# zju3dv/clean-pvnet

Measured on NVIDIA B200. Metric: ransac_vote_throughput, higher is better.
Workload: dtype f32

## Files before the change

### clean_pvnet_b200/_lib.py

```python
import ctypes
import os

_HERE = os.path.dirname(os.path.abspath(__file__))
LIB_PATH = os.path.join(_HERE, "libpvnet_vote_b200.so")

PVB_OK, PVB_ERR_INVALID, PVB_ERR_CUDA, PVB_ERR_WORKSPACE, PVB_ERR_CAPACITY, PVB_ERR_TIMEOUT = range(6)
PVB_HOST_STAGE_VERTEX, PVB_HOST_INPLACE_MASK = 2, 4
PVB_IPC_HANDLE_BYTES = 64
(PVB_MASK_U8, PVB_MASK_I8, PVB_MASK_I16, PVB_MASK_I32, PVB_MASK_I64, PVB_MASK_F32, PVB_MASK_F64) = range(7)
PVB_SELECT_BYTE, PVB_SELECT_EQ1 = 0, 1


class PvbDesc(ctypes.Structure):
    _fields_ = [
        ("B", ctypes.c_int32), ("H", ctypes.c_int32), ("W", ctypes.c_int32), ("K", ctypes.c_int32),
        ("hn", ctypes.c_int32),
        ("inlier_thresh", ctypes.c_float),
        ("min_num", ctypes.c_int32), ("max_num", ctypes.c_int32),
        ("mask_dtype", ctypes.c_int32), ("select_mode", ctypes.c_int32),
        ("mask_stride", ctypes.c_int64 * 3),
        ("vertex_stride", ctypes.c_int64 * 5),
        ("capacity", ctypes.c_int32), ("img_base", ctypes.c_int32),
        ("seed", ctypes.c_uint64),
        ("rng_tag_idx", ctypes.c_int32), ("rng_tag_sel", ctypes.c_int32),
    ]


class PvbLayout(ctypes.Structure):
    _fields_ = [(n, ctypes.c_size_t) for n in
                ("total", "status", "fgsum", "nz", "tn", "state", "bits", "ticket", "blocktot", "xy", "dirs", "hyp",
                 "counts", "win", "refit_partial", "refit_ticket")] + [
                    ("nwords", ctypes.c_int32), ("nblocks", ctypes.c_int32), ("capacity", ctypes.c_int32),
                    ("refit_splits", ctypes.c_int32)]


class PvbPnpOptions(ctypes.Structure):
    _fields_ = [("max_num_iterations", ctypes.c_int32), ("reserved", ctypes.c_int32),
                ("function_tolerance", ctypes.c_double), ("gradient_tolerance", ctypes.c_double),
                ("parameter_tolerance", ctypes.c_double)]


_vp, _i32, _sz, _f = ctypes.c_void_p, ctypes.c_int32, ctypes.c_size_t, ctypes.c_float
_dp, _lp = ctypes.POINTER(PvbDesc), ctypes.POINTER(PvbLayout)
SIGNATURES = {
    "pvb_version": (ctypes.c_int, []),
    "pvb_last_error": (ctypes.c_char_p, []),
    "pvb_workspace_bytes": (_sz, [_dp]),
    "pvb_workspace_layout": (ctypes.c_int, [_dp, _lp]),
    "pvb_ransac_voting_v3": (ctypes.c_int, [_dp, _vp, _vp, _vp, _vp, _vp, _vp, _sz, _vp]),
    "pvb_decode_v3": (ctypes.c_int, [_dp, _vp, _i32, ctypes.c_int64, _vp, _vp, _vp, _vp, _vp, _vp, _sz, _vp]),
    "pvb_estimate_voting_distribution": (ctypes.c_int, [_dp, _vp, _vp, _vp, _vp, _vp, _vp, _vp, _sz, _vp]),
    "pvb_uncertainty_weights": (ctypes.c_int, [_vp, _vp, _i32, _vp]),
    "pvb_uncertainty_pnp": (ctypes.c_int, [_vp, _vp, _vp, _vp, _vp, _vp, _vp, _i32, _i32, ctypes.c_int64, ctypes.c_int64,
                                           ctypes.c_void_p, _vp]),
    "pvb_uncertainty_pnp_from_votes": (ctypes.c_int, [_vp, _vp, _vp, _vp, _vp, _vp, _vp, _vp, _vp, _vp, _i32, _i32,
                                                      ctypes.c_int64, ctypes.c_int64, ctypes.c_void_p, _vp]),
    "pvb_uncertainty_pnp_init": (ctypes.c_int, [_vp, _vp, _vp, _vp, _vp, _i32, _i32, ctypes.c_int64, ctypes.c_int64, _vp]),
    "pvb_read_status": (ctypes.c_int, [_dp, _vp, _vp]),
    "pvb_host_scratch_bytes": (_sz, [_dp, _i32]),
    "pvb_ransac_voting_v3_host": (ctypes.c_int, [_dp, _vp, _vp, _vp, _i32, ctypes.c_uint32, _vp, _sz, _vp]),
    "pvb_exchange_create": (ctypes.c_int, [_i32, _i32, _i32, _sz, ctypes.POINTER(ctypes.c_void_p)]),
    "pvb_exchange_bytes_per_rank": (_sz, [_vp]),
    "pvb_exchange_base": (ctypes.c_void_p, [_vp]),
    "pvb_exchange_get_handle": (ctypes.c_int, [_vp, _vp]),
    "pvb_exchange_connect": (ctypes.c_int, [_vp, _vp]),
    "pvb_exchange_connect_ptrs": (ctypes.c_int, [_vp, ctypes.POINTER(ctypes.c_void_p)]),
    "pvb_ransac_voting_v3_push": (ctypes.c_int, [_dp, _vp, _vp, _vp, _vp, _vp, _vp, _sz, _vp, ctypes.c_uint64, _vp]),
    "pvb_estimate_voting_distribution_push": (ctypes.c_int, [_dp, _vp, _vp, _vp, _vp, _vp, _vp, _vp, _sz, _vp, ctypes.c_uint64, _vp]),
    "pvb_exchange_wait": (ctypes.c_int, [_vp, ctypes.c_uint64, _vp, _vp, ctypes.c_double, _vp]),
    "pvb_exchange_status": (ctypes.c_int, [_vp, _vp]),
    "pvb_exchange_destroy": (ctypes.c_int, [_vp]),
    "pvb_profile_enable": (ctypes.c_int, [_i32]),
    "pvb_profile_reset": (ctypes.c_int, []),
    "pvb_set_tuning": (ctypes.c_int, [_i32, _i32]),
    "pvb_profile_read": (ctypes.c_int, [ctypes.POINTER(ctypes.c_double), _i32]),
    "pvb_generate_hypothesis": (ctypes.c_int, [_vp, _vp, _vp, _vp, _i32, _i32, _i32, _vp]),
    "pvb_voting_for_hypothesis": (ctypes.c_int, [_vp, _vp, _vp, _vp, _i32, _i32, _i32, _f, _vp]),
    "pvb_generate_hypothesis_vanishing_point": (ctypes.c_int, [_vp, _vp, _vp, _vp, _i32, _i32, _i32, _vp]),
    "pvb_voting_for_hypothesis_vanishing_point": (ctypes.c_int, [_vp, _vp, _vp, _vp, _i32, _i32, _i32, _f, _vp]),
    "pvb_vote_count": (ctypes.c_int, [_vp, _vp, _vp, _vp, _i32, _i32, _i32, _f, _vp, _sz, _vp]),
    "pvb_vote_count_workspace_bytes": (_sz, [_i32, _i32, _i32]),
}

_LIB = None


def load():
    global _LIB
    if _LIB is None:
        if not os.path.exists(LIB_PATH):
            raise RuntimeError(
                f"{LIB_PATH} is missing: build it with `python clean_pvnet_b200/build.py` "
                "(or __graft_entry__.build()). There is no CPU/PyTorch fallback for this op.")
        lib = ctypes.CDLL(LIB_PATH)
        for name, (res, args) in SIGNATURES.items():
            fn = getattr(lib, name)
            fn.restype = res
            fn.argtypes = args
        _LIB = lib
        if os.environ.get("PVB_VOTE_VARIANT"):
            check(lib.pvb_set_tuning(0, int(os.environ["PVB_VOTE_VARIANT"])))
    return _LIB


def check(rc):
    if rc != PVB_OK:
        msg = load().pvb_last_error().decode("utf-8", "replace")
        raise RuntimeError(f"pvnet_vote_b200 error {rc}: {msg}")
```

### clean_pvnet_b200/csrc/api.cu

```cuda
#include <cmath>
#include <cstdarg>
#include <cstdio>
#include <cstring>
#include <new>
#include <vector>
#include "kernels.h"

using namespace pvb;

namespace {

thread_local char g_err[512] = "";

int fail(int code, const char *fmt, ...)
{
    va_list ap;
    va_start(ap, fmt);
    vsnprintf(g_err, sizeof(g_err), fmt, ap);
    va_end(ap);
    return code;
}

int cuda_fail(cudaError_t e, const char *what)
{
    return fail(PVB_ERR_CUDA, "%s: %s", what, cudaGetErrorString(e));
}

inline size_t align_up(size_t v, size_t a = 256) { return (v + a - 1) / a * a; }

struct ProfCall {
    cudaEvent_t ev[PVB_STAGE_COUNT + 1];
    bool head;
};
thread_local int g_prof_every = 0;
thread_local unsigned g_prof_tick = 0;
thread_local std::vector<ProfCall> g_prof_calls;
thread_local std::vector<cudaEvent_t> g_prof_pool;

cudaEvent_t prof_event()
{
    if (!g_prof_pool.empty()) { cudaEvent_t e = g_prof_pool.back(); g_prof_pool.pop_back(); return e; }
    cudaEvent_t e = nullptr;
    cudaEventCreate(&e);
    return e;
}

ProfCall *prof_begin(bool head)
{
    if (g_prof_every <= 0 || (g_prof_tick++ % (unsigned)g_prof_every) != 0) return nullptr;
    ProfCall pc;
    for (auto &e : pc.ev) e = prof_event();
    pc.head = head;
    g_prof_calls.push_back(pc);
    return &g_prof_calls.back();
}

inline void prof_start(ProfCall *pc, int stage, cudaStream_t st) { if (pc && stage == 0) cudaEventRecord(pc->ev[0], st); }
inline void prof_end(ProfCall *pc, int stage, cudaStream_t st) { if (pc) cudaEventRecord(pc->ev[stage + 1], st); }

int default_capacity(const pvb_desc *d)
{
    const long long HW = (long long)d->H * d->W;
    long long cap = d->capacity;
    if (cap <= 0) {
        const long long mn = d->max_num < 0 ? 0 : d->max_num;
        cap = mn + (long long)ceil(8.0 * sqrt((double)mn)) + 64;
    }
    if (cap > HW) cap = HW;
    cap = (cap + 31) / 32 * 32;
    return (int)cap;
}

int check_desc(const pvb_desc *d)
{
    if (!d) return fail(PVB_ERR_INVALID, "descriptor is NULL");
    if (d->B < 0 || d->H <= 0 || d->W <= 0 || d->K <= 0 || d->hn <= 0)
        return fail(PVB_ERR_INVALID, "bad shape B=%d H=%d W=%d K=%d hn=%d", d->B, d->H, d->W, d->K, d->hn);
    if ((long long)d->H * d->W > (1ll << 30)) return fail(PVB_ERR_INVALID, "image too large (H*W > 2^30)");
    if (d->B > 65535 || d->K > 65535) return fail(PVB_ERR_INVALID, "B and K must be <= 65535");
    if ((long long)d->K * ((d->hn + 511) / 512) > 65535) return fail(PVB_ERR_INVALID, "K*ceil(hn/512) must be <= 65535");
    if (d->mask_dtype < PVB_MASK_U8 || d->mask_dtype > PVB_MASK_F64) return fail(PVB_ERR_INVALID, "bad mask_dtype %d", d->mask_dtype);
    if (d->select_mode != PVB_SELECT_BYTE && d->select_mode != PVB_SELECT_EQ1)
        return fail(PVB_ERR_INVALID, "bad select_mode %d", d->select_mode);
    return PVB_OK;
}

int make_layout(const pvb_desc *d, pvb_layout *L)
{
    const int rc = check_desc(d);
    if (rc) return rc;
    const size_t B = (size_t)d->B, K = (size_t)d->K, hn = (size_t)d->hn;
    const int nwords = (int)(((long long)d->H * d->W + 31) / 32);
    const int nblocks = (nwords + 127) / 128;
    const int cap = default_capacity(d);
    const int splits = refit_splits_for(cap);
    size_t off = 0;
    auto take = [&](size_t bytes) { const size_t o = off; off = align_up(off + bytes); return o; };
    L->status = take(4 * sizeof(int));
    L->fgsum = take(B * sizeof(unsigned long long));
    L->nz = take(B * sizeof(int));
    L->tn = take(B * sizeof(int));
    L->state = take(B * sizeof(int));
    L->refit_ticket = take(B * K * sizeof(int));
    L->ticket = take(B * sizeof(int));
    L->blocktot = take(B * nblocks * sizeof(int));
    L->bits = take(B * nwords * sizeof(uint32_t));
    L->xy = take(B * cap * sizeof(float2));
    L->dirs = take(B * K * cap * sizeof(float2));
    L->hyp = take(B * K * hn * sizeof(float2));
    L->counts = take(B * K * hn * sizeof(int));
    L->win = take(B * K * sizeof(float2));
    L->refit_partial = take(B * K * splits * 5 * sizeof(double));
    L->total = off;
    L->nwords = nwords;
    L->nblocks = nblocks;
    L->capacity = cap;
    L->refit_splits = splits;
    return PVB_OK;
}

struct Plan {
    pvb_layout L;
    SelectArgs s;
    VoteArgs v;
    float2 *win;
    RefitScratch refit;
};

int make_plan(const pvb_desc *d, const void *mask, const float *vertex, const int32_t *idxs,
              const float *selection, void *ws, size_t ws_bytes, uint32_t tag_idx, uint32_t tag_sel, Plan *P)
{
    int rc = make_layout(d, &P->L);
    if (rc) return rc;
    if (!mask || !vertex) return fail(PVB_ERR_INVALID, "mask/vertex is NULL");
    if (!ws || ws_bytes < P->L.total) return fail(PVB_ERR_WORKSPACE, "workspace too small: need %zu bytes, got %zu", P->L.total, ws_bytes);
    if (reinterpret_cast<uintptr_t>(ws) & 255u) return fail(PVB_ERR_WORKSPACE, "workspace must be 256-byte aligned");
    char *w = static_cast<char *>(ws);
    const pvb_layout &L = P->L;
    SelectArgs &s = P->s;
    s.mask = mask; s.mask_dtype = d->mask_dtype; s.select_mode = d->select_mode;
    s.msb = d->mask_stride[0]; s.msy = d->mask_stride[1]; s.msx = d->mask_stride[2];
    s.vertex = vertex;
    for (int i = 0; i < 5; ++i) s.vs[i] = d->vertex_stride[i];
    s.selection = selection;
    s.B = d->B; s.H = d->H; s.W = d->W; s.K = d->K; s.nwords = L.nwords; s.nblocks = L.nblocks; s.cap = L.capacity;
    s.min_num = d->min_num; s.max_num = d->max_num; s.img_base = d->img_base;
    s.seed = d->seed; s.tag_sel = d->rng_tag_sel ? (uint32_t)d->rng_tag_sel : tag_sel;
    s.rowwise_gather = 0;
    s.seg_classes = 0; s.seg_cs = 0; s.mask_out = nullptr;
    s.bits = reinterpret_cast<uint32_t *>(w + L.bits);
    s.blocktot = reinterpret_cast<unsigned *>(w + L.blocktot);
    s.ticket = reinterpret_cast<int *>(w + L.ticket);
    s.fgsum = reinterpret_cast<unsigned long long *>(w + L.fgsum);
    s.nz = reinterpret_cast<int *>(w + L.nz);
    s.tn = reinterpret_cast<int *>(w + L.tn);
    s.state = reinterpret_cast<int *>(w + L.state);
    s.status = reinterpret_cast<int *>(w + L.status);
    s.xy = reinterpret_cast<float2 *>(w + L.xy);
    s.dirs = reinterpret_cast<float2 *>(w + L.dirs);
    VoteArgs &v = P->v;
    v.B = d->B; v.K = d->K; v.hn = d->hn; v.cap = L.capacity; v.W = d->W; v.H = d->H;
    v.thresh = d->inlier_thresh;
    v.tn = s.tn; v.state = s.state; v.xy = s.xy;
    v.dirs = s.dirs; v.idxs = idxs; v.seed = d->seed;
    v.tag_idx = d->rng_tag_idx ? (uint32_t)d->rng_tag_idx : tag_idx;
    v.img_base = d->img_base;
    v.hyp = reinterpret_cast<float2 *>(w + L.hyp);
    v.counts = reinterpret_cast<int *>(w + L.counts);
    P->win = reinterpret_cast<float2 *>(w + L.win);
    P->refit.partial = reinterpret_cast<double *>(w + L.refit_partial);
    P->refit.ticket = reinterpret_cast<int *>(w + L.refit_ticket);
    P->refit.splits = L.refit_splits;
    return PVB_OK;
}

int run_select(const Plan &P, cudaStream_t st)
{
    cudaError_t e = cudaMemsetAsync(P.s.status, 0, P.L.bits, st);
    if (e != cudaSuccess) return cuda_fail(e, "memset(header)");
    e = launch_select(P.s, st);
    if (e != cudaSuccess) return cuda_fail(e, "select kernels");
    return PVB_OK;
}

int run_front(const Plan &P, cudaStream_t st, ProfCall *pc)
{
    prof_start(pc, PVB_STAGE_SELECT, st);
    int rc = run_select(P, st);
    if (rc) return rc;
    prof_end(pc, PVB_STAGE_SELECT, st);
    prof_start(pc, PVB_STAGE_GENERATE, st);
    cudaError_t e = launch_generate(P.v, st);
    if (e != cudaSuccess) return cuda_fail(e, "generate kernel");
    prof_end(pc, PVB_STAGE_GENERATE, st);
    prof_start(pc, PVB_STAGE_VOTE, st);
    e = launch_vote(P.v, false, st);
    if (e != cudaSuccess) return cuda_fail(e, "vote kernel");
    prof_end(pc, PVB_STAGE_VOTE, st);
    return PVB_OK;
}

}

struct pvb_exchange {
    int rank, world, slots, device;
    size_t bytes_per_rank;
    size_t status_off, total;
    char *local;
    char *peer[PVB_MAX_PEERS];
    bool ipc_opened[PVB_MAX_PEERS];
    bool connected;
};

namespace {

int exchange_push_args(pvb_exchange *ex, uint64_t seq, size_t nbytes, PeerPush *pp)
{
    memset(pp, 0, sizeof(*pp));
    if (!ex) return PVB_OK;
    if (!ex->connected) return fail(PVB_ERR_INVALID, "exchange is not connected (pvb_exchange_connect*)");
    if (seq == 0 || (uint32_t)seq == 0) return fail(PVB_ERR_INVALID, "seq must be >= 1 and not a multiple of 2^32");
    if (nbytes > ex->bytes_per_rank) return fail(PVB_ERR_INVALID, "result block (%zu bytes) exceeds the exchange's bytes_per_rank (%zu)", nbytes, ex->bytes_per_rank);
    const size_t slot = (size_t)((seq - 1) % (uint64_t)ex->slots);
    const size_t words = ex->bytes_per_rank / sizeof(float);
    pp->world = ex->world;
    pp->seq = (uint32_t)seq;
    for (int r = 0; r < ex->world; ++r)
        pp->recv[r] = reinterpret_cast<uint2 *>(ex->peer[r]) + (slot * ex->world + ex->rank) * words;
    return PVB_OK;
}

size_t mask_elt_bytes(int dt)
{
    switch (dt) {
    case PVB_MASK_U8: case PVB_MASK_I8: return 1;
    case PVB_MASK_I16: return 2;
    case PVB_MASK_I32: case PVB_MASK_F32: return 4;
    default: return 8;
    }
}

}

extern "C" {

PVB_API int pvb_version(void) { return PVB_VERSION; }
PVB_API const char *pvb_last_error(void) { return g_err; }

PVB_API size_t pvb_workspace_bytes(const pvb_desc *d)
{
    pvb_layout L;
    if (make_layout(d, &L)) return 0;
    return L.total;
}

PVB_API int pvb_workspace_layout(const pvb_desc *d, pvb_layout *out)
{
    if (!out) return fail(PVB_ERR_INVALID, "out is NULL");
    return make_layout(d, out);
}

static int run_v3(const pvb_desc *d, const void *mask, const float *vertex, const int32_t *idxs, const float *selection,
                  float *out_kpt, void *workspace, size_t workspace_bytes, const float *seg, int32_t classes,
                  int64_t class_stride, int64_t *mask_out, pvb_exchange *ex, uint64_t seq, cudaStream_t st)
{
    Plan P;
    int rc = make_plan(d, seg ? static_cast<const void *>(seg) : mask, vertex, idxs, selection, workspace, workspace_bytes, 1u, 2u, &P);
    if (rc) return rc;
    if (!out_kpt) return fail(PVB_ERR_INVALID, "out_kpt is NULL");
    PeerPush pp;
    rc = exchange_push_args(ex, seq, (size_t)d->B * d->K * 2 * sizeof(float), &pp);
    if (rc) return rc;
    if (d->B == 0) {
        if (pp.world > 0) return fail(PVB_ERR_INVALID, "an exchanging call needs B >= 1 on every rank");
        return PVB_OK;
    }
    if (seg) {
        P.s.seg_classes = classes;
        P.s.seg_cs = class_stride;
        P.s.mask_out = reinterpret_cast<long long *>(mask_out);
    }
    ProfCall *pc = prof_begin(true);
    rc = run_front(P, st, pc);
    if (rc) return rc;
    prof_start(pc, PVB_STAGE_FINISH, st);
    cudaError_t e = launch_refit(P.v, P.win, P.refit, out_kpt, pp, st);
    if (e != cudaSuccess) return cuda_fail(e, "refit kernel");
    prof_end(pc, PVB_STAGE_FINISH, st);
    return PVB_OK;
}

PVB_API int pvb_ransac_voting_v3(const pvb_desc *d, const void *mask, const float *vertex, const int32_t *idxs,
                         const float *selection, float *out_kpt, void *workspace, size_t workspace_bytes,
                         pvb_stream_t stream)
{
    return run_v3(d, mask, vertex, idxs, selection, out_kpt, workspace, workspace_bytes, nullptr, 0, 0, nullptr, nullptr, 0,
                  static_cast<cudaStream_t>(stream));
}

PVB_API int pvb_ransac_voting_v3_push(const pvb_desc *d, const void *mask, const float *vertex, const int32_t *idxs,
                                      const float *selection, float *out_kpt, void *workspace, size_t workspace_bytes,
                                      pvb_exchange *exchange, uint64_t seq, pvb_stream_t stream)
{
    if (!exchange) return fail(PVB_ERR_INVALID, "exchange is NULL");
    return run_v3(d, mask, vertex, idxs, selection, out_kpt, workspace, workspace_bytes, nullptr, 0, 0, nullptr, exchange, seq,
                  static_cast<cudaStream_t>(stream));
}

PVB_API int pvb_decode_v3(const pvb_desc *d, const float *seg, int32_t classes, int64_t class_stride, int64_t *mask_out,
                          const float *vertex, const int32_t *idxs, const float *selection, float *out_kpt,
                          void *workspace, size_t workspace_bytes, pvb_stream_t stream)
{
    if (classes < 1 || classes > 4096) return fail(PVB_ERR_INVALID, "classes must be in [1,4096]");
    if (!seg) return fail(PVB_ERR_INVALID, "seg is NULL");
    return run_v3(d, nullptr, vertex, idxs, selection, out_kpt, workspace, workspace_bytes, seg, classes, class_stride, mask_out,
                  nullptr, 0, static_cast<cudaStream_t>(stream));
}

static int run_distribution(const pvb_desc *d, const void *mask, const float *vertex, const float *mean, const int32_t *idxs,
                            const float *selection, float *out_cov, void *workspace, size_t workspace_bytes, pvb_exchange *ex,
                            uint64_t seq, cudaStream_t st)
{
    Plan P;
    int rc = make_plan(d, mask, vertex, idxs, selection, workspace, workspace_bytes, 3u, 4u, &P);
    if (rc) return rc;
    if (!mean || !out_cov) return fail(PVB_ERR_INVALID, "mean/out_cov is NULL");
    PeerPush pp;
    rc = exchange_push_args(ex, seq, (size_t)d->B * d->K * 4 * sizeof(float), &pp);
    if (rc) return rc;
    if (d->B == 0) {
        if (pp.world > 0) return fail(PVB_ERR_INVALID, "an exchanging call needs B >= 1 on every rank");
        return PVB_OK;
    }
    ProfCall *pc = prof_begin(true);
    rc = run_front(P, st, pc);
    if (rc) return rc;
    prof_start(pc, PVB_STAGE_FINISH, st);
    cudaError_t e = launch_covariance(P.v, mean, out_cov, pp, st);
    if (e != cudaSuccess) return cuda_fail(e, "covariance kernel");
    prof_end(pc, PVB_STAGE_FINISH, st);
    return PVB_OK;
}

PVB_API int pvb_estimate_voting_distribution(const pvb_desc *d, const void *mask, const float *vertex, const float *mean,
                                     const int32_t *idxs, const float *selection, float *out_cov, void *workspace,
                                     size_t workspace_bytes, pvb_stream_t stream)
{
    return run_distribution(d, mask, vertex, mean, idxs, selection, out_cov, workspace, workspace_bytes, nullptr, 0,
                            static_cast<cudaStream_t>(stream));
}

PVB_API int pvb_estimate_voting_distribution_push(const pvb_desc *d, const void *mask, const float *vertex, const float *mean,
                                                  const int32_t *idxs, const float *selection, float *out_cov, void *workspace,
                                                  size_t workspace_bytes, pvb_exchange *exchange, uint64_t seq,
                                                  pvb_stream_t stream)
{
    if (!exchange) return fail(PVB_ERR_INVALID, "exchange is NULL");
    return run_distribution(d, mask, vertex, mean, idxs, selection, out_cov, workspace, workspace_bytes, exchange, seq,
                            static_cast<cudaStream_t>(stream));
}

PVB_API int pvb_uncertainty_weights(const float *cov, float *weights, int32_t n, pvb_stream_t stream)
{
    if (n < 0) return fail(PVB_ERR_INVALID, "n < 0");
    if (n && (!cov || !weights)) return fail(PVB_ERR_INVALID, "NULL tensor");
    if (reinterpret_cast<uintptr_t>(cov) & 15u) return fail(PVB_ERR_INVALID, "cov must be 16-byte aligned");
    cudaError_t e = launch_pnp_weights(cov, weights, n, static_cast<cudaStream_t>(stream));
    return e == cudaSuccess ? PVB_OK : cuda_fail(e, "pnp weights kernel");
}

PVB_API int pvb_uncertainty_pnp(const double *pts2d, const double *pts3d, const double *wgt2d, const double *K,
                                const double *init_rt, double *result_rt, int32_t *info, int32_t n, int32_t pn,
                                int64_t pts3d_stride, int64_t k_stride, const pvb_pnp_options *options, pvb_stream_t stream)
{
    if (n < 0) return fail(PVB_ERR_INVALID, "n < 0");
    if (pn < 1) return fail(PVB_ERR_INVALID, "pn must be >= 1 (got %d)", pn);
    if (n && (!pts2d || !pts3d || !wgt2d || !K || !init_rt || !result_rt)) return fail(PVB_ERR_INVALID, "NULL tensor");
    if (pts3d_stride < 0 || k_stride < 0) return fail(PVB_ERR_INVALID, "negative stride");
    PnpArgs a;
    a.pts2d = pts2d; a.pts3d = pts3d; a.wgt2d = wgt2d; a.K = K; a.init_rt = init_rt; a.result_rt = result_rt; a.info = info;
    a.n = n; a.pn = pn; a.pts3d_stride = pts3d_stride; a.k_stride = k_stride;
    a.max_num_iterations = 50; a.function_tolerance = 1e-6; a.gradient_tolerance = 1e-10; a.parameter_tolerance = 1e-8;
    if (options) {
        if (options->max_num_iterations < 0 || !(options->function_tolerance >= 0.0) || !(options->gradient_tolerance >= 0.0) ||
            !(options->parameter_tolerance >= 0.0))
            return fail(PVB_ERR_INVALID, "pvb_pnp_options: negative or NaN entry");
        a.max_num_iterations = options->max_num_iterations; a.function_tolerance = options->function_tolerance;
        a.gradient_tolerance = options->gradient_tolerance; a.parameter_tolerance = options->parameter_tolerance;
    }
    cudaError_t e = launch_pnp(a, static_cast<cudaStream_t>(stream));
    return e == cudaSuccess ? PVB_OK : cuda_fail(e, "uncertainty pnp kernel");
}

PVB_API int pvb_uncertainty_pnp_from_votes(const float *kpt_2d, const float *cov, const float *weights, const double *pts3d,
                                           const double *K, const double *init_rt, double *result_rt, double *init_out,
                                           float *weights_out, int32_t *info, int32_t n, int32_t pn, int64_t pts3d_stride,
                                           int64_t k_stride, const pvb_pnp_options *options, pvb_stream_t stream)
{
    if (n < 0) return fail(PVB_ERR_INVALID, "n < 0");
    if (pn < 1 || pn > PNP_FUSED_MAX_PN) return fail(PVB_ERR_INVALID, "pn must be in [1,%d] (got %d)", PNP_FUSED_MAX_PN, pn);
    if (!init_rt && pn < 4) return fail(PVB_ERR_INVALID, "the P3P initialisation needs pn >= 4 (got %d)", pn);
    if (n && (!kpt_2d || !pts3d || !K || !result_rt)) return fail(PVB_ERR_INVALID, "NULL tensor");
    if (n && ((cov == nullptr) == (weights == nullptr))) return fail(PVB_ERR_INVALID, "pass exactly one of cov / weights");
    if (pts3d_stride < 0 || k_stride < 0) return fail(PVB_ERR_INVALID, "negative stride");
    if ((reinterpret_cast<uintptr_t>(kpt_2d) & 7u) || (reinterpret_cast<uintptr_t>(cov) & 15u))
        return fail(PVB_ERR_INVALID, "kpt_2d must be 8-byte and cov 16-byte aligned");
    PnpFusedArgs a;
    a.kpt2d = kpt_2d; a.cov = cov; a.weights = weights; a.pts3d = pts3d; a.K = K; a.init_rt = init_rt; a.result_rt = result_rt;
    a.init_out = init_out; a.weights_out = weights_out; a.info = info; a.n = n; a.pn = pn;
    a.pts3d_stride = pts3d_stride; a.k_stride = k_stride;
    a.max_num_iterations = 50; a.function_tolerance = 1e-6; a.gradient_tolerance = 1e-10; a.parameter_tolerance = 1e-8;
    if (options) {
        if (options->max_num_iterations < 0 || !(options->function_tolerance >= 0.0) || !(options->gradient_tolerance >= 0.0) ||
            !(options->parameter_tolerance >= 0.0))
            return fail(PVB_ERR_INVALID, "pvb_pnp_options: negative or NaN entry");
        a.max_num_iterations = options->max_num_iterations; a.function_tolerance = options->function_tolerance;
        a.gradient_tolerance = options->gradient_tolerance; a.parameter_tolerance = options->parameter_tolerance;
    }
    cudaError_t e = launch_pnp_fused(a, static_cast<cudaStream_t>(stream));
    return e == cudaSuccess ? PVB_OK : cuda_fail(e, "fused uncertainty pnp kernel");
}

PVB_API int pvb_uncertainty_pnp_init(const double *pts2d, const double *pts3d, const double *wgt2d, const double *K,
                                     double *init_rt, int32_t n, int32_t pn, int64_t pts3d_stride, int64_t k_stride,
                                     pvb_stream_t stream)
{
    if (n < 0) return fail(PVB_ERR_INVALID, "n < 0");
    if (pn < 4) return fail(PVB_ERR_INVALID, "P3P needs pn >= 4 (got %d)", pn);
    if (n && (!pts2d || !pts3d || !wgt2d || !K || !init_rt)) return fail(PVB_ERR_INVALID, "NULL tensor");
    if (pts3d_stride < 0 || k_stride < 0) return fail(PVB_ERR_INVALID, "negative stride");
    PnpArgs a;
    a.pts2d = pts2d; a.pts3d = pts3d; a.wgt2d = wgt2d; a.K = K; a.init_rt = nullptr; a.result_rt = init_rt; a.info = nullptr;
    a.n = n; a.pn = pn; a.pts3d_stride = pts3d_stride; a.k_stride = k_stride;
    a.max_num_iterations = 0; a.function_tolerance = a.gradient_tolerance = a.parameter_tolerance = 0.0;
    cudaError_t e = launch_p3p_init(a, static_cast<cudaStream_t>(stream));
    return e == cudaSuccess ? PVB_OK : cuda_fail(e, "p3p init kernel");
}

PVB_API int pvb_read_status(const pvb_desc *d, const void *workspace, pvb_stream_t stream)
{
    pvb_layout L;
    int rc = make_layout(d, &L);
    if (rc) return rc;
    if (!workspace) return fail(PVB_ERR_INVALID, "workspace is NULL");
    int host[4] = {0, 0, 0, 0};
    cudaStream_t st = static_cast<cudaStream_t>(stream);
    cudaError_t e = cudaMemcpyAsync(host, static_cast<const char *>(workspace) + L.status, sizeof(host), cudaMemcpyDeviceToHost, st);
    if (e == cudaSuccess) e = cudaStreamSynchronize(st);
    if (e != cudaSuccess) return cuda_fail(e, "read status");
    if (host[0] == PVB_ERR_CAPACITY)
        return fail(PVB_ERR_CAPACITY, "image %d selected more than capacity=%d pixels; pass capacity=H*W", host[1], L.capacity);
    if (host[0]) return fail(host[0], "device status %d", host[0]);
    return PVB_OK;
}

struct HostSlot { size_t mask, vertex, out, ws, end; };

static int host_slot_layout(const pvb_desc *d, int chunk, HostSlot *S, pvb_desc *dc)
{
    if (chunk <= 0) return fail(PVB_ERR_INVALID, "chunk_images must be > 0");
    *dc = *d;
    dc->B = chunk;
    const size_t HW = (size_t)d->H * d->W;
    dc->mask_stride[0] = (int64_t)HW; dc->mask_stride[1] = d->W; dc->mask_stride[2] = 1;
    dc->vertex_stride[0] = (int64_t)(HW * d->K * 2); dc->vertex_stride[1] = (int64_t)d->W * d->K * 2;
    dc->vertex_stride[2] = (int64_t)d->K * 2; dc->vertex_stride[3] = 2; dc->vertex_stride[4] = 1;
    pvb_layout L;
    int rc = make_layout(dc, &L);
    if (rc) return rc;
    size_t off = 0;
    S->mask = off; off = align_up(off + (size_t)chunk * HW * mask_elt_bytes(d->mask_dtype));
    S->vertex = off; off = align_up(off + (size_t)chunk * HW * d->K * 2 * sizeof(float));
    S->out = off; off = align_up(off + (size_t)chunk * d->K * 2 * sizeof(float));
    S->ws = off; off = align_up(off + L.total);
    S->end = off;
    return PVB_OK;
}

constexpr int HOST_SLOTS = 4;

PVB_API size_t pvb_host_scratch_bytes(const pvb_desc *d, int32_t chunk_images)
{
    HostSlot S; pvb_desc dc;
    if (check_desc(d) || host_slot_layout(d, chunk_images, &S, &dc)) return 0;
    return HOST_SLOTS * S.end;
}

namespace {
struct HostPipe {
    cudaStream_t copy = nullptr, in = nullptr, cmp = nullptr;
    cudaEvent_t user = nullptr, end = nullptr, dma[HOST_SLOTS] = {}, sel[HOST_SLOTS] = {}, done[HOST_SLOTS] = {};
    bool ready = false;
};
constexpr int MAX_DEVICES = 64;

int host_pipe(int dev, HostPipe **out)
{
    static thread_local HostPipe pipes[MAX_DEVICES];
    if (dev < 0 || dev >= MAX_DEVICES) return fail(PVB_ERR_CUDA, "device index %d out of range", dev);
    HostPipe &p = pipes[dev];
    if (!p.ready) {
        int lo = 0, hi = 0;
        cudaDeviceGetStreamPriorityRange(&lo, &hi);
        cudaError_t e = cudaStreamCreateWithPriority(&p.copy, cudaStreamNonBlocking, hi);
        if (e == cudaSuccess) e = cudaStreamCreateWithPriority(&p.in, cudaStreamNonBlocking, hi);
        if (e == cudaSuccess) e = cudaStreamCreateWithPriority(&p.cmp, cudaStreamNonBlocking, lo);
        if (e != cudaSuccess) return cuda_fail(e, "cudaStreamCreate");
        cudaEvent_t *single[] = {&p.user, &p.end};
        for (cudaEvent_t *pe : single)
            if ((e = cudaEventCreateWithFlags(pe, cudaEventDisableTiming)) != cudaSuccess) return cuda_fail(e, "cudaEventCreate");
        for (int i = 0; i < HOST_SLOTS; ++i) {
            e = cudaEventCreateWithFlags(&p.dma[i], cudaEventDisableTiming);
            if (e == cudaSuccess) e = cudaEventCreateWithFlags(&p.sel[i], cudaEventDisableTiming);
            if (e == cudaSuccess) e = cudaEventCreateWithFlags(&p.done[i], cudaEventDisableTiming);
            if (e != cudaSuccess) return cuda_fail(e, "cudaEventCreate");
        }
        p.ready = true;
    }
    *out = &p;
    return PVB_OK;
}

const void *mapped_alias(const void *p)
{
    cudaPointerAttributes a;
    if (cudaPointerGetAttributes(&a, p) != cudaSuccess) { cudaGetLastError(); return nullptr; }
    if (a.type != cudaMemoryTypeHost || !a.devicePointer) return nullptr;
    return a.devicePointer;
}
}

PVB_API int pvb_ransac_voting_v3_host(const pvb_desc *d, const void *mask_host, const float *vertex_host,
                              float *out_kpt_host, int32_t chunk_images, uint32_t flags, void *dev_scratch,
                              size_t dev_scratch_bytes, pvb_stream_t stream)
{
    int rc = check_desc(d);
    if (rc) return rc;
    if (!mask_host || !vertex_host || !out_kpt_host) return fail(PVB_ERR_INVALID, "host buffer is NULL");
    if (flags & ~(uint32_t)(PVB_HOST_INPLACE_MASK | PVB_HOST_STAGE_VERTEX)) return fail(PVB_ERR_INVALID, "unknown flags 0x%x", flags);
    HostSlot S; pvb_desc dc;
    rc = host_slot_layout(d, chunk_images, &S, &dc);
    if (rc) return rc;
    if (!dev_scratch || dev_scratch_bytes < HOST_SLOTS * S.end) return fail(PVB_ERR_WORKSPACE, "device scratch too small: need %zu", HOST_SLOTS * S.end);
    if (reinterpret_cast<uintptr_t>(dev_scratch) & 255u) return fail(PVB_ERR_WORKSPACE, "device scratch must be 256-byte aligned");
    int dev = 0;
    cudaError_t e = cudaGetDevice(&dev);
    if (e != cudaSuccess) return cuda_fail(e, "cudaGetDevice");
    HostPipe *hp = nullptr;
    rc = host_pipe(dev, &hp);
    if (rc) return rc;
    cudaStream_t user = static_cast<cudaStream_t>(stream);
    e = cudaEventRecord(hp->user, user);
    if (e == cudaSuccess) e = cudaStreamWaitEvent(hp->copy, hp->user, 0);
    if (e == cudaSuccess) e = cudaStreamWaitEvent(hp->in, hp->user, 0);
    if (e == cudaSuccess) e = cudaStreamWaitEvent(hp->cmp, hp->user, 0);
    if (e != cudaSuccess) return cuda_fail(e, "stream wait");
    const size_t HW = (size_t)d->H * d->W;
    const size_t mbytes = HW * mask_elt_bytes(d->mask_dtype), vbytes = HW * d->K * 2 * sizeof(float);
    const size_t obytes = (size_t)d->K * 2 * sizeof(float);
    char *base = static_cast<char *>(dev_scratch);
    pvb_layout Lc;
    rc = make_layout(&dc, &Lc);
    if (rc) return rc;
    const char *mask_alias = static_cast<const char *>(mapped_alias(mask_host));
    const char *vertex_alias = static_cast<const char *>(mapped_alias(vertex_host));
    const bool stage_mask = !(flags & PVB_HOST_INPLACE_MASK) || !mask_alias;
    const bool stage_vertex = (flags & PVB_HOST_STAGE_VERTEX) || !vertex_alias;
    int piece = 0;
    for (int b0 = 0; b0 < d->B; b0 += chunk_images, ++piece) {
        const int slot = piece % HOST_SLOTS;
        const int c = (d->B - b0 < chunk_images) ? d->B - b0 : chunk_images;
        char *sb = base + (size_t)slot * S.end;
        const void *mptr = sb + S.mask;
        const float *vptr = reinterpret_cast<const float *>(sb + S.vertex);
        if (piece >= HOST_SLOTS) {
            e = cudaStreamWaitEvent(hp->copy, hp->done[slot], 0);
            if (e == cudaSuccess) e = cudaStreamWaitEvent(hp->in, hp->done[slot], 0);
            if (e != cudaSuccess) return cuda_fail(e, "stream wait");
        }
        if (stage_mask)
            e = cudaMemcpyAsync(sb + S.mask, static_cast<const char *>(mask_host) + (size_t)b0 * mbytes, (size_t)c * mbytes, cudaMemcpyHostToDevice, hp->copy);
        else
            mptr = mask_alias + (size_t)b0 * mbytes;
        if (e == cudaSuccess && stage_vertex)
            e = cudaMemcpyAsync(sb + S.vertex, reinterpret_cast<const char *>(vertex_host) + (size_t)b0 * vbytes, (size_t)c * vbytes, cudaMemcpyHostToDevice, hp->copy);
        else if (e == cudaSuccess)
            vptr = reinterpret_cast<const float *>(vertex_alias + (size_t)b0 * vbytes);
        if (e != cudaSuccess) return cuda_fail(e, "H2D copy");
        if (stage_mask || stage_vertex) {
            e = cudaEventRecord(hp->dma[slot], hp->copy);
            if (e == cudaSuccess) e = cudaStreamWaitEvent(hp->in, hp->dma[slot], 0);
            if (e != cudaSuccess) return cuda_fail(e, "pipeline event");
        }
        pvb_desc di = dc;
        di.B = c;
        di.img_base = d->img_base + b0;
        di.capacity = Lc.capacity;
        Plan P;
        rc = make_plan(&di, mptr, vptr, nullptr, nullptr, sb + S.ws, S.end - S.ws, 1u, 2u, &P);
        if (rc) return rc;
        P.s.rowwise_gather = stage_vertex ? 0 : 1;
        rc = run_select(P, hp->in);
        if (rc) return rc;
        e = cudaEventRecord(hp->sel[slot], hp->in);
        if (e == cudaSuccess) e = cudaStreamWaitEvent(hp->cmp, hp->sel[slot], 0);
        if (e != cudaSuccess) return cuda_fail(e, "pipeline event");
        PeerPush none;
        memset(&none, 0, sizeof(none));
        e = launch_generate(P.v, hp->cmp);
        if (e == cudaSuccess) e = launch_vote(P.v, false, hp->cmp);
        if (e == cudaSuccess) e = launch_refit(P.v, P.win, P.refit, reinterpret_cast<float *>(sb + S.out), none, hp->cmp);
        if (e != cudaSuccess) return cuda_fail(e, "compute kernels");
        e = cudaMemcpyAsync(reinterpret_cast<char *>(out_kpt_host) + (size_t)b0 * obytes, sb + S.out, (size_t)c * obytes, cudaMemcpyDeviceToHost, hp->cmp);
        if (e == cudaSuccess) e = cudaEventRecord(hp->done[slot], hp->cmp);
        if (e != cudaSuccess) return cuda_fail(e, "D2H copy");
    }
    e = cudaEventRecord(hp->end, hp->cmp);
    if (e == cudaSuccess) e = cudaStreamWaitEvent(user, hp->end, 0);
    if (e == cudaSuccess) e = cudaStreamSynchronize(user);
    if (e != cudaSuccess) return cuda_fail(e, "stream sync");
    return PVB_OK;
}

PVB_API int pvb_profile_enable(int32_t every) { g_prof_every = every < 0 ? 0 : every; g_prof_tick = 0; return PVB_OK; }

PVB_API int pvb_set_tuning(int32_t gather_mode, int32_t vote_variant)
{
    if (vote_variant < 0 || vote_variant > 3) return fail(PVB_ERR_INVALID, "vote_variant must be 0..3");
    if (gather_mode < 0 || gather_mode > 2) return fail(PVB_ERR_INVALID, "gather_mode must be 0..2");
    set_gather_tuning(gather_mode);
    set_vote_tuning(vote_variant);
    return PVB_OK;
}

PVB_API int pvb_profile_reset(void)
{
    for (auto &pc : g_prof_calls)
        for (auto e : pc.ev) g_prof_pool.push_back(e);
    g_prof_calls.clear();
    return PVB_OK;
}

PVB_API int pvb_profile_read(double *ms, int32_t n)
{
    if (!ms || n < PVB_STAGE_COUNT) return fail(PVB_ERR_INVALID, "ms must hold PVB_STAGE_COUNT doubles");
    int calls = 0;
    for (auto &pc : g_prof_calls) {
        for (int i = 0; i < PVB_STAGE_COUNT; ++i) {
            cudaError_t e = cudaEventSynchronize(pc.ev[i + 1]);
            float t = 0.f;
            if (e == cudaSuccess) e = cudaEventElapsedTime(&t, pc.ev[i], pc.ev[i + 1]);
            if (e != cudaSuccess) { cuda_fail(e, "profile elapsed"); return -1; }
            ms[i] += (double)t;
        }
        if (pc.head) ++calls;
    }
    pvb_profile_reset();
    return calls;
}

static int check_compat(const void *a, const void *b, const void *c, const void *d_, int tn, int vn, int hn)
{
    if (tn < 0 || vn < 0 || hn < 0) return fail(PVB_ERR_INVALID, "negative size");
    if ((long long)hn * vn > (1ll << 30) || (long long)tn * vn > (1ll << 30)) return fail(PVB_ERR_INVALID, "problem too large");
    if (((tn && vn) && (!a || !b)) || ((hn && vn) && (!c || !d_))) return fail(PVB_ERR_INVALID, "NULL tensor");
    if (vn > 65535) return fail(PVB_ERR_INVALID, "vn must be <= 65535");
    return PVB_OK;
}

PVB_API int pvb_generate_hypothesis(const float *direct, const float *coords, const int32_t *idxs, float *hyp, int32_t tn,
                            int32_t vn, int32_t hn, pvb_stream_t stream)
{
    int rc = check_compat(direct, coords, idxs, hyp, tn, vn, hn);
    if (rc) return rc;
    cudaError_t e = launch_compat_generate(direct, coords, idxs, hyp, tn, vn, hn, false, static_cast<cudaStream_t>(stream));
    return e == cudaSuccess ? PVB_OK : cuda_fail(e, "generate_hypothesis");
}

PVB_API int pvb_generate_hypothesis_vanishing_point(const float *direct, const float *coords, const int32_t *idxs, float *hyp,
                                            int32_t tn, int32_t vn, int32_t hn, pvb_stream_t stream)
{
    int rc = check_compat(direct, coords, idxs, hyp, tn, vn, hn);
    if (rc) return rc;
    cudaError_t e = launch_compat_generate(direct, coords, idxs, hyp, tn, vn, hn, true, static_cast<cudaStream_t>(stream));
    return e == cudaSuccess ? PVB_OK : cuda_fail(e, "generate_hypothesis_vanishing_point");
}

PVB_API int pvb_voting_for_hypothesis(const float *direct, const float *coords, const float *hyp, uint8_t *inliers, int32_t tn,
                              int32_t vn, int32_t hn, float inlier_thresh, pvb_stream_t stream)
{
    int rc = check_compat(direct, coords, hyp, inliers, tn, vn, hn);
    if (rc) return rc;
    if (tn && vn && hn && !inliers) return fail(PVB_ERR_INVALID, "NULL tensor");
    cudaError_t e = launch_compat_vote(direct, coords, hyp, inliers, tn, vn, hn, inlier_thresh, false, static_cast<cudaStream_t>(stream));
    return e == cudaSuccess ? PVB_OK : cuda_fail(e, "voting_for_hypothesis");
}

PVB_API int pvb_voting_for_hypothesis_vanishing_point(const float *direct, const float *coords, const float *hyp,
                                              uint8_t *inliers, int32_t tn, int32_t vn, int32_t hn,
                                              float inlier_thresh, pvb_stream_t stream)
{
    int rc = check_compat(direct, coords, hyp, inliers, tn, vn, hn);
    if (rc) return rc;
    if (tn && vn && hn && !inliers) return fail(PVB_ERR_INVALID, "NULL tensor");
    cudaError_t e = launch_compat_vote(direct, coords, hyp, inliers, tn, vn, hn, inlier_thresh, true, static_cast<cudaStream_t>(stream));
    return e == cudaSuccess ? PVB_OK : cuda_fail(e, "voting_for_hypothesis_vanishing_point");
}

PVB_API size_t pvb_vote_count_workspace_bytes(int32_t tn, int32_t vn, int32_t hn)
{
    if (tn < 0 || vn < 0 || hn < 0) return 0;
    size_t off = align_up(4 * sizeof(int));
    off += align_up((size_t)tn * sizeof(float2));
    off += align_up((size_t)tn * vn * sizeof(float2));
    off += align_up((size_t)hn * vn * sizeof(float2));
    off += align_up((size_t)hn * vn * sizeof(int));
    return off;
}

PVB_API int pvb_vote_count(const float *direct, const float *coords, const float *hyp, int32_t *counts, int32_t tn, int32_t vn,
                   int32_t hn, float inlier_thresh, void *workspace, size_t workspace_bytes, pvb_stream_t stream)
{
    int rc = check_compat(direct, coords, hyp, counts, tn, vn, hn);
    if (rc) return rc;
    cudaStream_t st = static_cast<cudaStream_t>(stream);
    if (hn == 0 || vn == 0) return PVB_OK;
    if (tn == 0) {
        cudaError_t e = cudaMemsetAsync(counts, 0, sizeof(int) * (size_t)hn * vn, st);
        return e == cudaSuccess ? PVB_OK : cuda_fail(e, "memset");
    }
    if ((long long)vn * ((hn + 511) / 512) > 65535) return fail(PVB_ERR_INVALID, "vn*ceil(hn/512) must be <= 65535");
    const size_t need = pvb_vote_count_workspace_bytes(tn, vn, hn);
    if (!workspace || workspace_bytes < need) return fail(PVB_ERR_WORKSPACE, "workspace too small: need %zu", need);
    if (reinterpret_cast<uintptr_t>(workspace) & 255u) return fail(PVB_ERR_WORKSPACE, "workspace must be 256-byte aligned");
    char *w = static_cast<char *>(workspace);
    size_t off = 0;
    int *meta = reinterpret_cast<int *>(w + off); off += align_up(4 * sizeof(int));
    float2 *xy = reinterpret_cast<float2 *>(w + off); off += align_up((size_t)tn * sizeof(float2));
    float2 *dirs = reinterpret_cast<float2 *>(w + off); off += align_up((size_t)tn * vn * sizeof(float2));
    float2 *hyp_k = reinterpret_cast<float2 *>(w + off); off += align_up((size_t)hn * vn * sizeof(float2));
    int *counts_k = reinterpret_cast<int *>(w + off);
    cudaError_t e = launch_compat_repack(direct, coords, hyp, tn, vn, hn, dirs, xy, hyp_k, meta, st);
    if (e != cudaSuccess) return cuda_fail(e, "repack");
    VoteArgs v;
    memset(&v, 0, sizeof(v));
    v.B = 1; v.K = vn; v.hn = hn; v.cap = tn; v.W = 0; v.H = 0; v.thresh = inlier_thresh;
    v.tn = meta; v.state = meta + 1; v.xy = xy;
    v.dirs = dirs; v.idxs = nullptr; v.hyp = hyp_k; v.counts = counts_k;
    e = launch_vote(v, true, st);
    if (e != cudaSuccess) return cuda_fail(e, "vote kernel");
    e = launch_compat_unpack_counts(counts_k, counts, vn, hn, st);
    return e == cudaSuccess ? PVB_OK : cuda_fail(e, "unpack");
}

PVB_API int pvb_exchange_create(int32_t rank, int32_t world, int32_t slots, size_t bytes_per_rank, pvb_exchange **out)
{
    if (!out) return fail(PVB_ERR_INVALID, "out is NULL");
    *out = nullptr;
    if (world < 1 || world > PVB_MAX_PEERS || rank < 0 || rank >= world) return fail(PVB_ERR_INVALID, "bad rank %d / world %d (max %d)", rank, world, PVB_MAX_PEERS);
    if (slots < 2 || slots > 4096) return fail(PVB_ERR_INVALID, "slots must be in [2,4096]");
    if (bytes_per_rank == 0 || bytes_per_rank > ((size_t)1 << 30)) return fail(PVB_ERR_INVALID, "bad bytes_per_rank");
    pvb_exchange *ex = new (std::nothrow) pvb_exchange();
    if (!ex) return fail(PVB_ERR_INVALID, "out of host memory");
    memset(ex, 0, sizeof(*ex));
    ex->rank = rank; ex->world = world; ex->slots = slots;
    ex->bytes_per_rank = (bytes_per_rank + 15) / 16 * 16;
    ex->status_off = align_up((size_t)slots * world * ex->bytes_per_rank * 2);
    ex->total = ex->status_off + 256;
    cudaError_t e = cudaGetDevice(&ex->device);
    if (e == cudaSuccess) e = cudaMalloc(reinterpret_cast<void **>(&ex->local), ex->total);
    if (e == cudaSuccess) e = cudaMemset(ex->local, 0, ex->total);
    if (e == cudaSuccess) e = cudaDeviceSynchronize();
    if (e != cudaSuccess) { if (ex->local) cudaFree(ex->local); delete ex; return cuda_fail(e, "exchange allocation"); }
    ex->peer[rank] = ex->local;
    ex->connected = (world == 1);
    *out = ex;
    return PVB_OK;
}

PVB_API size_t pvb_exchange_bytes_per_rank(const pvb_exchange *ex) { return ex ? ex->bytes_per_rank : 0; }
PVB_API void *pvb_exchange_base(const pvb_exchange *ex) { return ex ? ex->local : nullptr; }

PVB_API int pvb_exchange_get_handle(const pvb_exchange *ex, void *handle)
{
    if (!ex || !handle) return fail(PVB_ERR_INVALID, "NULL argument");
    static_assert(sizeof(cudaIpcMemHandle_t) == PVB_IPC_HANDLE_BYTES, "handle size");
    cudaIpcMemHandle_t h;
    cudaError_t e = cudaIpcGetMemHandle(&h, ex->local);
    if (e != cudaSuccess) return cuda_fail(e, "cudaIpcGetMemHandle");
    memcpy(handle, &h, sizeof(h));
    return PVB_OK;
}

PVB_API int pvb_exchange_connect_ptrs(pvb_exchange *ex, void *const *bases)
{
    if (!ex || !bases) return fail(PVB_ERR_INVALID, "NULL argument");
    for (int r = 0; r < ex->world; ++r) {
        if (r == ex->rank) continue;
        if (!bases[r]) return fail(PVB_ERR_INVALID, "base pointer of rank %d is NULL", r);
        ex->peer[r] = static_cast<char *>(bases[r]);
    }
    ex->connected = true;
    return PVB_OK;
}

PVB_API int pvb_exchange_connect(pvb_exchange *ex, const void *handles)
{
    if (!ex || !handles) return fail(PVB_ERR_INVALID, "NULL argument");
    const char *hb = static_cast<const char *>(handles);
    for (int r = 0; r < ex->world; ++r) {
        if (r == ex->rank || ex->ipc_opened[r]) continue;
        cudaIpcMemHandle_t h;
        memcpy(&h, hb + (size_t)r * PVB_IPC_HANDLE_BYTES, sizeof(h));
        void *p = nullptr;
        cudaError_t e = cudaIpcOpenMemHandle(&p, h, cudaIpcMemLazyEnablePeerAccess);
        if (e != cudaSuccess) return cuda_fail(e, "cudaIpcOpenMemHandle (peer memory over NVLink needs P2P access between the GPUs)");
        ex->peer[r] = static_cast<char *>(p);
        ex->ipc_opened[r] = true;
    }
    ex->connected = true;
    return PVB_OK;
}

PVB_API int pvb_exchange_wait(pvb_exchange *ex, uint64_t seq, void *out, const int32_t *floats_per_rank, double timeout_s,
                              pvb_stream_t stream)
{
    if (!ex || !out) return fail(PVB_ERR_INVALID, "NULL argument");
    if (seq == 0 || (uint32_t)seq == 0) return fail(PVB_ERR_INVALID, "seq must be >= 1 and not a multiple of 2^32");
    if (reinterpret_cast<uintptr_t>(out) & 3u) return fail(PVB_ERR_INVALID, "out must be 4-byte aligned");
    if (!(timeout_s > 0.0)) timeout_s = 10.0;
    const int words = (int)(ex->bytes_per_rank / sizeof(float));
    ExchangeCounts counts;
    for (int r = 0; r < PVB_MAX_PEERS; ++r) counts.n[r] = 0;
    for (int r = 0; r < ex->world; ++r) {
        const int n = floats_per_rank ? floats_per_rank[r] : words;
        if (n < 0 || n > words) return fail(PVB_ERR_INVALID, "floats_per_rank[%d] = %d outside [0, %d]", r, n, words);
        counts.n[r] = n;
    }
    const size_t slot = (size_t)((seq - 1) % (uint64_t)ex->slots);
    const uint2 *recv = reinterpret_cast<const uint2 *>(ex->local) + slot * ex->world * words;
    cudaError_t e = launch_exchange_wait(recv, (uint32_t)seq, static_cast<float *>(out), ex->world, words, counts,
                                         (unsigned long long)(timeout_s * 1e9), reinterpret_cast<int *>(ex->local + ex->status_off),
                                         static_cast<cudaStream_t>(stream));
    return e == cudaSuccess ? PVB_OK : cuda_fail(e, "exchange wait kernel");
}

PVB_API int pvb_exchange_status(pvb_exchange *ex, pvb_stream_t stream)
{
    if (!ex) return fail(PVB_ERR_INVALID, "NULL argument");
    int host = 0;
    cudaStream_t st = static_cast<cudaStream_t>(stream);
    cudaError_t e = cudaMemcpyAsync(&host, ex->local + ex->status_off, sizeof(int), cudaMemcpyDeviceToHost, st);
    if (e == cudaSuccess) e = cudaStreamSynchronize(st);
    if (e != cudaSuccess) return cuda_fail(e, "exchange status");
    if (host) return fail(PVB_ERR_TIMEOUT, "a pvb_exchange_wait timed out: some rank never published its result");
    return PVB_OK;
}

PVB_API int pvb_exchange_destroy(pvb_exchange *ex)
{
    if (!ex) return PVB_OK;
    cudaDeviceSynchronize();
    for (int r = 0; r < ex->world; ++r)
        if (ex->ipc_opened[r]) cudaIpcCloseMemHandle(ex->peer[r]);
    if (ex->local) cudaFree(ex->local);
    delete ex;
    return PVB_OK;
}

}
```

### clean_pvnet_b200/csrc/kernels.h

```cpp
#pragma once
#include <cuda_runtime.h>
#include <stdint.h>
#include "../../include/pvnet_vote_b200.h"

namespace pvb {

struct SelectArgs {
    const void *mask;
    int mask_dtype, select_mode;
    long long msb, msy, msx;
    const float *vertex;
    long long vs[5];
    const float *selection;
    int B, H, W, K, nwords, nblocks, cap, min_num, max_num, img_base;
    int rowwise_gather;
    int seg_classes;
    long long seg_cs;
    long long *mask_out;
    uint64_t seed;
    uint32_t tag_sel;
    uint32_t *bits;
    unsigned *blocktot;
    int *ticket;
    unsigned long long *fgsum;
    int *nz, *tn, *state, *status;
    float2 *xy, *dirs;
};
cudaError_t launch_select(const SelectArgs &a, cudaStream_t st);

struct VoteArgs {
    int B, K, hn, cap, W, H;
    float thresh;
    const int *tn;
    const int *state;
    const float2 *xy;
    const float2 *dirs;
    const int32_t *idxs;
    uint64_t seed;
    uint32_t tag_idx;
    int img_base;
    float2 *hyp;
    int *counts;
};
cudaError_t launch_generate(const VoteArgs &a, cudaStream_t st);
cudaError_t launch_vote(const VoteArgs &a, bool zero_counts, cudaStream_t st);
void set_vote_tuning(int variant);
void set_gather_tuning(int mode);
struct RefitScratch { double *partial; int *ticket; int splits; };
int refit_splits_for(int cap);
constexpr int PVB_MAX_PEERS = 16;
struct PeerPush {
    int world;
    unsigned int seq;
    uint2 *recv[PVB_MAX_PEERS];
};
cudaError_t launch_refit(const VoteArgs &a, float2 *win, const RefitScratch &rs, float *out_kpt, const PeerPush &pp,
                         cudaStream_t st);
struct ExchangeCounts { int n[PVB_MAX_PEERS]; };
cudaError_t launch_exchange_wait(const uint2 *recv, unsigned int seq, float *out, int world, int stride_words,
                                 const ExchangeCounts &counts, unsigned long long timeout_ns, int *status, cudaStream_t st);
cudaError_t launch_covariance(const VoteArgs &a, const float *mean, float *out_cov, const PeerPush &pp, cudaStream_t st);

cudaError_t launch_pnp_weights(const float *cov, float *w, int n, cudaStream_t st);

struct PnpArgs {
    const double *pts2d;
    const double *pts3d;
    const double *wgt2d;
    const double *K;
    const double *init_rt;
    double *result_rt;
    int *info;
    int n, pn;
    long long pts3d_stride, k_stride;
    int max_num_iterations;
    double function_tolerance, gradient_tolerance, parameter_tolerance;
};
cudaError_t launch_pnp(const PnpArgs &a, cudaStream_t st);
cudaError_t launch_p3p_init(const PnpArgs &a, cudaStream_t st);

constexpr int PNP_FUSED_MAX_PN = 64;
struct PnpFusedArgs {
    const float *kpt2d;
    const float *cov;
    const float *weights;
    const double *pts3d;
    const double *K;
    const double *init_rt;
    double *result_rt;
    double *init_out;
    float *weights_out;
    int *info;
    int n, pn;
    long long pts3d_stride, k_stride;
    int max_num_iterations;
    double function_tolerance, gradient_tolerance, parameter_tolerance;
};
cudaError_t launch_pnp_fused(const PnpFusedArgs &a, cudaStream_t st);

cudaError_t launch_compat_generate(const float *direct, const float *coords, const int32_t *idxs, float *hyp,
                                   int tn, int vn, int hn, bool vanishing, cudaStream_t st);
cudaError_t launch_compat_vote(const float *direct, const float *coords, const float *hyp, uint8_t *inliers,
                               int tn, int vn, int hn, float thresh, bool vanishing, cudaStream_t st);
cudaError_t launch_compat_repack(const float *direct, const float *coords, const float *hyp, int tn, int vn,
                                 int hn, float2 *dirs, float2 *xy, float2 *hyp_k, int *meta, cudaStream_t st);
cudaError_t launch_compat_unpack_counts(const int *counts_k, int *counts, int vn, int hn, cudaStream_t st);

}
```

### clean_pvnet_b200/csrc/vote.cu

```cuda
#include <atomic>
#include <math_constants.h>
#include "common.cuh"
#include "kernels.h"

namespace pvb {

__global__ void __launch_bounds__(256)
generate_kernel(VoteArgs a)
{
    const int h = blockIdx.x * 256 + threadIdx.x;
    if (h >= a.hn) return;
    const int k = blockIdx.y, b = blockIdx.z;
    const int tn = min(a.tn[b], a.cap);
    float x = 0.f, y = 0.f;
    if (tn > 0) {
        int t0, t1;
        if (a.idxs) {
            const int2 t = __ldg(reinterpret_cast<const int2 *>(a.idxs) + ((size_t)b * a.hn + h) * a.K + k);
            t0 = t.x; t1 = t.y;
        } else {
            const uint4 r = philox4x32_10(make_uint4((uint32_t)h, (uint32_t)k, (uint32_t)(a.img_base + b), a.tag_idx),
                                          make_uint2((uint32_t)a.seed, (uint32_t)(a.seed >> 32)));
            t0 = (int)(r.x % (uint32_t)tn);
            t1 = (int)(r.y % (uint32_t)tn);
        }
        if ((unsigned)t0 < (unsigned)tn && (unsigned)t1 < (unsigned)tn) {
            const float2 *dk = a.dirs + ((size_t)b * a.K + k) * a.cap;
            const float2 *xy = a.xy + (size_t)b * a.cap;
            const float2 d0 = dk[t0], d1 = dk[t1], c0 = xy[t0], c1 = xy[t1];
            float hx, hy;
            if (hypothesis_from_pair(d0.x, d0.y, c0.x, c0.y, d1.x, d1.y, c1.x, c1.y, hx, hy)) { x = hx; y = hy; }
        }
    }
    a.hyp[((size_t)b * a.K + k) * a.hn + h] = make_float2(x, y);
    a.counts[((size_t)b * a.K + k) * a.hn + h] = 0;
}

cudaError_t launch_generate(const VoteArgs &a, cudaStream_t st)
{
    dim3 g((a.hn + 255) / 256, a.K, a.B);
    generate_kernel<<<g, 256, 0, st>>>(a);
    return cudaGetLastError();
}

struct VoteK {
    VoteArgs a;
    ConeParams cone;
};

constexpr int VOTE_BLOCK = 16;

__device__ __forceinline__ float4 lds128(uint32_t addr)
{
    float4 v;
    asm volatile("ld.shared.v4.f32 {%0,%1,%2,%3}, [%4];" : "=f"(v.x), "=f"(v.y), "=f"(v.z), "=f"(v.w) : "r"(addr) : "memory");
    return v;
}

__device__ __forceinline__ float cone_margin(const float4 ra, const float2 rb, float hxc, float hyc)
{
    const float ap = fmaf(ra.x, hxc, fmaf(ra.y, hyc, ra.z));
    const float pp = fmaf(ra.w, hxc, fmaf(rb.x, hyc, rb.y));
    return ap - fabsf(pp);
}

template <int HPT, int NT, int MINB, int VOTE_TILE, int WS>
__global__ void __launch_bounds__(NT, MINB)
vote_kernel(const VoteK p)
{
    constexpr int PPT = VOTE_TILE / NT;
    constexpr int NW = NT / 32;
    constexpr int TEAM = WS * 32;
    constexpr int TEAMS = NT / TEAM;
    __shared__ __align__(16) float4 s_a[VOTE_TILE];
    __shared__ __align__(16) float2 s_b[VOTE_TILE];
    __shared__ float s_box[4][NW];
    const VoteArgs &a = p.a;
    const int b = blockIdx.z;
    const int k = blockIdx.y % a.K, slice = blockIdx.y / a.K;
    const int tn = min(a.tn[b], a.cap);
    const int t0 = blockIdx.x * VOTE_TILE;
    if (t0 >= tn) return;
    const int n = min(VOTE_TILE, tn - t0);
    const int npad = (n + VOTE_BLOCK - 1) / VOTE_BLOCK * VOTE_BLOCK;
    const int tid = threadIdx.x, lane = tid & 31, warp = tid >> 5;
    const float kappa = p.cone.kappa, thresh = p.cone.thresh;
    const float2 *hyp = a.hyp + ((size_t)b * a.K + k) * a.hn;
    const float2 *xy = a.xy + (size_t)b * a.cap + t0;
    const float2 *dk = a.dirs + ((size_t)b * a.K + k) * a.cap + t0;
    const int team = tid / TEAM;
    const int hbase = slice * (TEAM * HPT) + (tid - team * TEAM);

    float2 v[PPT], c[PPT];
    float x0 = CUDART_INF_F, x1 = -CUDART_INF_F, y0 = CUDART_INF_F, y1 = -CUDART_INF_F;
#pragma unroll
    for (int r = 0; r < PPT; ++r) {
        const int i = tid + r * NT;
        v[r] = make_float2(0.f, 0.f); c[r] = make_float2(0.f, 0.f);
        if (i < n) {
            v[r] = __ldg(dk + i); c[r] = __ldg(xy + i);
            x0 = fminf(x0, c[r].x); x1 = fmaxf(x1, c[r].x); y0 = fminf(y0, c[r].y); y1 = fmaxf(y1, c[r].y);
        }
    }
#pragma unroll
    for (int o = 16; o > 0; o >>= 1) {
        x0 = fminf(x0, __shfl_xor_sync(0xffffffffu, x0, o)); x1 = fmaxf(x1, __shfl_xor_sync(0xffffffffu, x1, o));
        y0 = fminf(y0, __shfl_xor_sync(0xffffffffu, y0, o)); y1 = fmaxf(y1, __shfl_xor_sync(0xffffffffu, y1, o));
    }
    if (lane == 0) { s_box[0][warp] = x0; s_box[1][warp] = x1; s_box[2][warp] = y0; s_box[3][warp] = y1; }
    __syncthreads();
#pragma unroll
    for (int w = 0; w < NW; ++w) {
        x0 = fminf(x0, s_box[0][w]); x1 = fmaxf(x1, s_box[1][w]); y0 = fminf(y0, s_box[2][w]); y1 = fmaxf(y1, s_box[3][w]);
    }
    const float ox = 0.5f * (x0 + x1), oy = 0.5f * (y0 + y1);
    const float cmax = (0.5f * (x1 - x0) + 0.5f * (y1 - y0)) * 1.000001f + 1e-3f;

#pragma unroll
    for (int r = 0; r < PPT; ++r) {
        const int i = tid + r * NT;
        if (i < npad) {
            float4 ra = make_float4(0.f, 0.f, -1e30f, 0.f);
            float2 rb = make_float2(0.f, 0.f);
            if (i < n) {
                const float n1 = __fsqrt_rn(__fmaf_rn(v[r].x, v[r].x, __fmul_rn(v[r].y, v[r].y)));
                const float cxc = c[r].x - ox, cyc = c[r].y - oy;
                if (!(n1 > below_1e6())) {
                } else if (!(n1 < 1e18f) || !(fabsf(cxc) + fabsf(cyc) <= cmax)) {
                    ra.z = 0.f;
                } else {
                    const float inv = 1.0f / n1;
                    const float ux = v[r].x * inv, uy = v[r].y * inv;
                    const float a1 = kappa * ux, a2 = kappa * uy;
                    ra.x = a1; ra.y = a2; ra.z = -fmaf(a1, cxc, a2 * cyc);
                    ra.w = -uy; rb.x = ux; rb.y = fmaf(uy, cxc, -(ux * cyc));
                }
            }
            s_a[i] = ra; s_b[i] = rb;
        }
    }

    float hxc[HPT], hyc[HPT], dl[HPT];
    int neg[HPT];
#pragma unroll
    for (int j = 0; j < HPT; ++j) {
        const int h = hbase + j * TEAM;
        const float2 q = (h < a.hn) ? hyp[h] : make_float2(0.f, 0.f);
        float xc = q.x - ox, yc = q.y - oy;
        const float S = fabsf(xc) + fabsf(yc) + cmax;
        float d = fmaxf(p.cone.band * S, 1e-30f);
        if (!(S <= 1e15f) || !(d < CUDART_INF_F)) { xc = 0.f; yc = 0.f; d = CUDART_INF_F; }
        hxc[j] = xc; hyc[j] = yc; dl[j] = d;
        neg[j] = 0;
    }
    __syncthreads();

    const uint32_t sa0 = (uint32_t)__cvta_generic_to_shared(s_a);
    const uint32_t sb0 = (uint32_t)__cvta_generic_to_shared(s_b);
    int mine = 0;
    for (int i0 = team * VOTE_BLOCK; i0 < npad; i0 += TEAMS * VOTE_BLOCK) {
        mine += VOTE_BLOCK;
        const uint32_t sa = sa0 + (uint32_t)i0 * 16u, sb = sb0 + (uint32_t)i0 * 8u;
        float mn[HPT];
#pragma unroll
        for (int j = 0; j < HPT; ++j) mn[j] = CUDART_INF_F;
#pragma unroll
        for (int u = 0; u < VOTE_BLOCK; u += 2) {
            const float4 ra0 = lds128(sa + u * 16), ra1 = lds128(sa + u * 16 + 16);
            const float4 rbb = lds128(sb + u * 8);
#pragma unroll
            for (int j = 0; j < HPT; ++j) {
                const float m0 = cone_margin(ra0, make_float2(rbb.x, rbb.y), hxc[j], hyc[j]);
                const float m1 = cone_margin(ra1, make_float2(rbb.z, rbb.w), hxc[j], hyc[j]);
                neg[j] += (int)(__float_as_uint(m0) >> 31);
                neg[j] += (int)(__float_as_uint(m1) >> 31);
                mn[j] = fminf(mn[j], fminf(fabsf(m0), fabsf(m1)));
            }
        }
        bool flag = false;
#pragma unroll
        for (int j = 0; j < HPT; ++j) flag |= mn[j] < dl[j];
        if (__any_sync(0xffffffffu, flag)) {
            const int nb = min(VOTE_BLOCK, n - i0);
            float4 ra = make_float4(0.f, 0.f, -1e30f, 0.f);
            float2 rb = make_float2(0.f, 0.f), vv = make_float2(0.f, 0.f), cc = make_float2(0.f, 0.f);
            if (lane < nb) {
                ra = s_a[i0 + lane]; rb = s_b[i0 + lane];
                vv = __ldg(dk + i0 + lane); cc = __ldg(xy + i0 + lane);
            }
#pragma unroll
            for (int j = 0; j < HPT; ++j) {
                unsigned bm = __ballot_sync(0xffffffffu, mn[j] < dl[j]);
                while (bm) {
                    const int L = __ffs(bm) - 1;
                    bm &= bm - 1;
                    const float hx_ = __shfl_sync(0xffffffffu, hxc[j], L), hy_ = __shfl_sync(0xffffffffu, hyc[j], L);
                    const float dl_ = __shfl_sync(0xffffffffu, dl[j], L);
                    const int h = hbase - lane + L + j * TEAM;
                    const float2 q = (h < a.hn) ? __ldg(hyp + h) : make_float2(0.f, 0.f);
                    int delta = 0;
                    if (lane < nb) {
                        const float m = cone_margin(ra, rb, hx_, hy_);
                        if (fabsf(m) < dl_) {
                            const bool in = vote_exact(vv.x, vv.y, cc.x, cc.y, q.x, q.y, thresh);
                            delta = (in ? 0 : 1) - (int)(__float_as_uint(m) >> 31);
                        }
                    }
                    delta = __reduce_add_sync(0xffffffffu, delta);
                    if (lane == L) neg[j] += delta;
                }
            }
        }
    }
    int *counts = a.counts + ((size_t)b * a.K + k) * a.hn;
#pragma unroll
    for (int j = 0; j < HPT; ++j) {
        const int h = hbase + j * TEAM;
        const int cnt = mine - neg[j];
        if (h < a.hn && cnt) atomicAdd(counts + h, cnt);
    }
}

ConeParams make_cone(float thresh)
{
    ConeParams c;
    c.thresh = thresh;
    const double t = (double)thresh;
    if (t > 0.0 && t < 1.0) {
        const double s = sqrt(1.0 - t * t);
        const double kappa = s / t, G = 1.0 / (t * s);
        const double band = 1.25 * ldexp(1.0, -24) * (18.0 + 22.0 * kappa + 9.0 * G);
        c.kappa = (float)kappa;
        c.band = nextafterf((float)band, INFINITY);
    } else {
        c.kappa = 0.f;
        c.band = INFINITY;
    }
    return c;
}

static std::atomic<int> g_vote_variant{0};

void set_vote_tuning(int variant) { g_vote_variant.store(variant, std::memory_order_relaxed); }

cudaError_t launch_vote(const VoteArgs &a, bool zero_counts, cudaStream_t st)
{
    if (zero_counts) {
        cudaError_t e = cudaMemsetAsync(a.counts, 0, sizeof(int) * (size_t)a.B * a.K * a.hn, st);
        if (e != cudaSuccess) return e;
    }
    VoteK p;
    p.a = a;
    p.cone = make_cone(a.thresh);
    const int variant = g_vote_variant.load(std::memory_order_relaxed);
#define PVB_VOTE(HPT, NT, MINB, TILE, WS)                                               \
    do {                                                                                \
        const int slices = (a.hn + (HPT) * (WS) * 32 - 1) / ((HPT) * (WS) * 32);        \
        dim3 g((a.cap + (TILE) - 1) / (TILE), a.K * slices, a.B);                       \
        vote_kernel<HPT, NT, MINB, TILE, WS><<<g, NT, 0, st>>>(p);                      \
    } while (0)
    if (a.hn <= 32) PVB_VOTE(1, 128, 8, 512, 1);
    else if (a.hn <= 64) PVB_VOTE(2, 128, 8, 512, 1);
    else if (a.hn <= 128) PVB_VOTE(4, 128, 8, 512, 1);
    else if (a.hn <= 256) PVB_VOTE(4, 128, 8, 512, 2);
    else if (variant == 2) PVB_VOTE(4, 128, 8, 256, 4);
    else if (variant == 3) PVB_VOTE(4, 128, 8, 1024, 4);
    else PVB_VOTE(4, 128, 8, 512, 4);
#undef PVB_VOTE
    return cudaGetLastError();
}

template <int NV>
__device__ __forceinline__ void peer_push(const PeerPush &pp, size_t bk, const float (&v)[NV])
{
    for (int r = 0; r < pp.world; ++r) {
        uint2 *dst = pp.recv[r] + bk * NV;
#pragma unroll
        for (int i = 0; i < NV; ++i)
            asm volatile("st.volatile.global.v2.u32 [%0], {%1, %2};" ::"l"(dst + i), "r"(__float_as_uint(v[i])), "r"(pp.seq) : "memory");
    }
}

constexpr int RF_THREADS = 128;
constexpr int RF_CHUNK = 2048;

int refit_splits_for(int cap) { return (cap + RF_CHUNK - 1) / RF_CHUNK; }

__device__ __forceinline__ bool vote_winner(float vx, float vy, float cx, float cy, float hx, float hy,
                                            const ConeParams &cone)
{
    const float dx = __fsub_rn(hx, cx), dy = __fsub_rn(hy, cy);
    const float n1sq = fmaf(vx, vx, vy * vy);
    const float S = fabsf(dx) + fabsf(dy);
    const float m = cone.kappa * fmaf(vx, dx, vy * dy) - fabsf(fmaf(vx, dy, -(vy * dx)));
    const float thr = cone.band * S;
    const bool safe = (n1sq > 1e-10f) && (n1sq < 1e8f) && (S <= 1e6f) && (m * m > thr * thr * n1sq * 1.0001f);
    return safe ? (m > 0.f) : vote_exact(vx, vy, cx, cy, hx, hy, cone.thresh);
}

__global__ void __launch_bounds__(RF_THREADS)
refit_kernel(VoteArgs a, float2 *__restrict__ win, RefitScratch rs, float *__restrict__ out, ConeParams cone, PeerPush pp)
{
    const int split = blockIdx.x, k = blockIdx.y, b = blockIdx.z;
    const int tid = threadIdx.x, lane = tid & 31, warp = tid >> 5;
    constexpr int NW = RF_THREADS / 32;
    const int tn = min(a.tn[b], a.cap);
    const size_t bk = (size_t)b * a.K + k;
    __shared__ int s_c[NW], s_h[NW];
    __shared__ double s_acc[NW][5];
    __shared__ int s_last;
    float2 res = make_float2(0.f, 0.f);
    if (a.state[b] != 0 || tn <= 0) {
        if (split != 0) return;
        if (tid == 0) { out[bk * 2] = 0.f; out[bk * 2 + 1] = 0.f; win[bk] = make_float2(0.f, 0.f); }
    } else {
        const int nsplit = (tn + RF_CHUNK - 1) / RF_CHUNK;
        if (split >= nsplit) return;
        const int *counts = a.counts + bk * a.hn;
        int bc = -1, bh = 0x7fffffff;
        for (int h = tid; h < a.hn; h += RF_THREADS) {
            const int c = counts[h];
            if (c > bc) { bc = c; bh = h; }
        }
#pragma unroll
        for (int o = 16; o > 0; o >>= 1) {
            const int oc = __shfl_xor_sync(0xffffffffu, bc, o), oh = __shfl_xor_sync(0xffffffffu, bh, o);
            if (oc > bc || (oc == bc && oh < bh)) { bc = oc; bh = oh; }
        }
        if (lane == 0) { s_c[warp] = bc; s_h[warp] = bh; }
        __syncthreads();
#pragma unroll
        for (int w = 0; w < NW; ++w)
            if (s_c[w] > bc || (s_c[w] == bc && s_h[w] < bh)) { bc = s_c[w]; bh = s_h[w]; }
        const float2 wpt = (bc > 0) ? a.hyp[bk * a.hn + bh] : make_float2(0.f, 0.f);
        if (split == 0 && tid == 0) win[bk] = wpt;

        const float2 *xy = a.xy + (size_t)b * a.cap;
        const float2 *dk = a.dirs + bk * a.cap;
        const int t_end = min(tn, (split + 1) * RF_CHUNK);
        double a00 = 0, a01 = 0, a11 = 0, b0 = 0, b1 = 0;
        constexpr int RU = 4;
        for (int t0 = split * RF_CHUNK + tid; t0 < t_end; t0 += RF_THREADS * RU) {
            float2 v[RU], c[RU];
#pragma unroll
            for (int u = 0; u < RU; ++u) {
                const int t = t0 + u * RF_THREADS;
                v[u] = make_float2(0.f, 0.f); c[u] = make_float2(0.f, 0.f);
                if (t < t_end) { v[u] = __ldg(dk + t); c[u] = __ldg(xy + t); }
            }
#pragma unroll
            for (int u = 0; u < RU; ++u) {
                if (t0 + u * RF_THREADS < t_end && vote_winner(v[u].x, v[u].y, c[u].x, c[u].y, wpt.x, wpt.y, cone)) {
                    const double nx = (double)v[u].y, ny = -(double)v[u].x;
                    const double bb = nx * (double)c[u].x + ny * (double)c[u].y;
                    a00 += nx * nx; a01 += nx * ny; a11 += ny * ny;
                    b0 += nx * bb; b1 += ny * bb;
                }
            }
        }
        a00 = warp_sum(a00); a01 = warp_sum(a01); a11 = warp_sum(a11); b0 = warp_sum(b0); b1 = warp_sum(b1);
        if (lane == 0) { s_acc[warp][0] = a00; s_acc[warp][1] = a01; s_acc[warp][2] = a11; s_acc[warp][3] = b0; s_acc[warp][4] = b1; }
        __syncthreads();
        if (tid == 0) {
            double *pq = rs.partial + (bk * rs.splits + split) * 5;
            for (int i = 0; i < 5; ++i) {
                double s = 0;
                for (int w = 0; w < NW; ++w) s += s_acc[w][i];
                __stcg(pq + i, s);
            }
            __threadfence();
            s_last = (atomicAdd(rs.ticket + bk, 1) == nsplit - 1);
        }
        __syncthreads();
        if (!s_last) return;
        if (tid == 0) {
            __threadfence();
            double s[5] = {0, 0, 0, 0, 0};
            for (int sp = 0; sp < nsplit; ++sp)
                for (int i = 0; i < 5; ++i) s[i] += __ldcg(rs.partial + (bk * rs.splits + sp) * 5 + i);
            const double det = s[0] * s[2] - s[1] * s[1];
            float x, y;
            if (det == 0.0 || !isfinite(det)) { x = (float)s[3]; y = (float)s[4]; }
            else { x = (float)((s[2] * s[3] - s[1] * s[4]) / det); y = (float)((s[0] * s[4] - s[1] * s[3]) / det); }
            out[bk * 2] = x; out[bk * 2 + 1] = y;
            res = make_float2(x, y);
        }
    }
    if (pp.world <= 0 || tid != 0) return;
    const float v[2] = {res.x, res.y};
    peer_push<2>(pp, bk, v);
}

cudaError_t launch_refit(const VoteArgs &a, float2 *win, const RefitScratch &rs, float *out_kpt, const PeerPush &pp,
                         cudaStream_t st)
{
    dim3 g(rs.splits, a.K, a.B);
    refit_kernel<<<g, RF_THREADS, 0, st>>>(a, win, rs, out_kpt, make_cone(a.thresh), pp);
    return cudaGetLastError();
}

constexpr int CV_THREADS = 256;

__global__ void __launch_bounds__(CV_THREADS)
covariance_kernel(VoteArgs a, const float *__restrict__ mean, float *__restrict__ cov, PeerPush pp)
{
    const int k = blockIdx.x, b = blockIdx.y;
    const int tid = threadIdx.x, lane = tid & 31, warp = tid >> 5;
    const size_t bk = (size_t)b * a.K + k;
    const int tn = min(a.tn[b], a.cap);
    const bool skipped = a.state[b] != 0;
    const int *counts = a.counts + bk * a.hn;
    const float2 *hyp = a.hyp + bk * a.hn;
    const float ftn = (float)tn;
    __shared__ float s_max[CV_THREADS / 32];
    __shared__ double s_acc[CV_THREADS / 32][4];
    float mx = -CUDART_INF_F;
    bool has_nan = false;
    for (int h = tid; h < a.hn; h += CV_THREADS) {
        const float r = skipped ? 1.f : __fdiv_rn((float)counts[h], ftn);
        if (r != r) has_nan = true;
        mx = fmaxf(mx, r);
    }
#pragma unroll
    for (int o = 16; o > 0; o >>= 1) mx = fmaxf(mx, __shfl_xor_sync(0xffffffffu, mx, o));
    if (lane == 0) s_max[warp] = mx;
    __syncthreads();
    mx = s_max[0];
    for (int w = 1; w < CV_THREADS / 32; ++w) mx = fmaxf(mx, s_max[w]);
    (void)has_nan;
    const float th = __fsub_rn(mx, 0.1f);
    const float mx_ = mean[bk * 2], my_ = mean[bk * 2 + 1];
    double s00 = 0, s01 = 0, s11 = 0, sw = 0;
    for (int h = tid; h < a.hn; h += CV_THREADS) {
        float w = skipped ? 1.f : __fdiv_rn((float)counts[h], ftn);
        if (w < th) w = 0.f;
        const float2 q = skipped ? make_float2(0.f, 0.f) : hyp[h];
        const double dx = (double)__fsub_rn(q.x, mx_), dy = (double)__fsub_rn(q.y, my_);
        s00 += dx * (dx * w); s01 += dx * (dy * w); s11 += dy * (dy * w); sw += w;
    }
    s00 = warp_sum(s00); s01 = warp_sum(s01); s11 = warp_sum(s11); sw = warp_sum(sw);
    if (lane == 0) { s_acc[warp][0] = s00; s_acc[warp][1] = s01; s_acc[warp][2] = s11; s_acc[warp][3] = sw; }
    __syncthreads();
    if (tid == 0) {
        double s[4] = {0, 0, 0, 0};
        for (int w = 0; w < CV_THREADS / 32; ++w)
            for (int i = 0; i < 4; ++i) s[i] += s_acc[w][i];
        const double den = (double)__fadd_rn((float)s[3], 1e-3f);
        float *c = cov + bk * 4;
        const float v[4] = {(float)(s[0] / den), (float)(s[1] / den), (float)(s[1] / den), (float)(s[2] / den)};
        c[0] = v[0]; c[1] = v[1]; c[2] = v[2]; c[3] = v[3];
        if (pp.world > 0) peer_push<4>(pp, bk, v);
    }
}

cudaError_t launch_covariance(const VoteArgs &a, const float *mean, float *out_cov, const PeerPush &pp, cudaStream_t st)
{
    dim3 g(a.K, a.B);
    covariance_kernel<<<g, CV_THREADS, 0, st>>>(a, mean, out_cov, pp);
    return cudaGetLastError();
}

__global__ void __launch_bounds__(128)
pnp_weights_kernel(const float *__restrict__ cov, float *__restrict__ w, int n)
{
    const int i = blockIdx.x * 128 + threadIdx.x;
    if (i >= n) return;
    float o0, o1, o2;
    cov_to_weights(__ldg(reinterpret_cast<const float4 *>(cov) + i), o0, o1, o2);
    w[(size_t)i * 3] = o0; w[(size_t)i * 3 + 1] = o1; w[(size_t)i * 3 + 2] = o2;
}

cudaError_t launch_pnp_weights(const float *cov, float *w, int n, cudaStream_t st)
{
    if (n <= 0) return cudaSuccess;
    pnp_weights_kernel<<<(n + 127) / 128, 128, 0, st>>>(cov, w, n);
    return cudaGetLastError();
}

}
```

### clean_pvnet_b200/ransac_voting_gpu.py

```python
import math
import sys
import types

import torch

from . import _lib
from . import ransac_voting as _ext

_MASK_DTYPES = {
    torch.uint8: _lib.PVB_MASK_U8, torch.bool: _lib.PVB_MASK_U8, torch.int8: _lib.PVB_MASK_I8,
    torch.int16: _lib.PVB_MASK_I16, torch.int32: _lib.PVB_MASK_I32, torch.int64: _lib.PVB_MASK_I64,
    torch.float32: _lib.PVB_MASK_F32, torch.float64: _lib.PVB_MASK_F64,
}

_workspaces = {}
_VALIDATE_CAPACITY = True


def _workspace(device, nbytes):
    key = (device.index, torch.cuda.current_stream(device).cuda_stream)
    ws = _workspaces.get(key)
    if ws is None or ws.numel() < nbytes:
        ws = torch.empty(int(nbytes * 1.25) + 256, dtype=torch.uint8, device=device)
        _workspaces[key] = ws
    return ws


def _draw_seed():
    return int(torch.empty((), dtype=torch.int64).random_().item()) & 0xFFFFFFFFFFFFFFFF


def _check_inputs(mask, vertex):
    if not isinstance(mask, torch.Tensor) or not mask.is_cuda:
        raise RuntimeError("mask must be a CUDA tensor")
    if not isinstance(vertex, torch.Tensor) or not vertex.is_cuda:
        raise RuntimeError("vertex must be a CUDA tensor")
    if vertex.dim() != 5 or vertex.size(4) != 2:
        raise RuntimeError("vertex must be [b,h,w,vn,2]")
    if mask.dim() != 3 or tuple(mask.shape) != tuple(vertex.shape[:3]):
        raise RuntimeError("mask must be [b,h,w] matching vertex")
    if mask.device != vertex.device:
        raise RuntimeError("mask and vertex must be on the same device")
    if vertex.dtype != torch.float32:
        vertex = vertex.float()
    if mask.dtype in (torch.float16, torch.bfloat16):
        mask = mask.float()
    if mask.dtype not in _MASK_DTYPES:
        raise RuntimeError(f"unsupported mask dtype {mask.dtype}")
    return mask, vertex


_desc_cache = {}


def _cached_desc(lib, mask, vertex, hn, inlier_thresh, min_num, max_num, select_mode, seed, img_base, capacity):
    key = (mask.dtype, mask.stride(), tuple(vertex.shape), vertex.stride(), hn, float(inlier_thresh), min_num, max_num,
           select_mode, capacity)
    hit = _desc_cache.get(key)
    if hit is None:
        d = _make_desc(mask, vertex, hn, inlier_thresh, min_num, max_num, select_mode, 0, 0, capacity)
        nbytes = lib.pvb_workspace_bytes(d)
        if nbytes == 0:
            _lib.check(lib.pvb_workspace_layout(d, _lib.PvbLayout()))
        if len(_desc_cache) > 64:
            _desc_cache.clear()
        hit = _desc_cache[key] = (d, nbytes)
    d, nbytes = hit
    d.seed = int(seed) & 0xFFFFFFFFFFFFFFFF
    d.img_base = int(img_base)
    return d, nbytes


def _make_desc(mask, vertex, hn, inlier_thresh, min_num, max_num, select_mode, seed, img_base, capacity):
    d = _lib.PvbDesc()
    d.B, d.H, d.W, d.K = vertex.size(0), vertex.size(1), vertex.size(2), vertex.size(3)
    d.hn = int(hn)
    d.inlier_thresh = float(inlier_thresh)
    d.min_num, d.max_num = int(min_num), int(min(max_num, 2 ** 31 - 1))
    d.mask_dtype = _MASK_DTYPES[mask.dtype]
    d.select_mode = select_mode
    for i in range(3):
        d.mask_stride[i] = mask.stride(i)
    for i in range(5):
        d.vertex_stride[i] = vertex.stride(i)
    d.capacity = int(capacity or 0)
    d.img_base = int(img_base)
    d.seed = int(seed) & 0xFFFFFFFFFFFFFFFF
    return d


def _views(ws, d, lib):
    L = _lib.PvbLayout()
    _lib.check(lib.pvb_workspace_layout(d, L))
    B, K, hn, cap = d.B, d.K, d.hn, L.capacity

    def view(off, count, dtype):
        nbytes = count * torch.empty((), dtype=dtype).element_size()
        return ws[off:off + nbytes].view(dtype)

    out = dict(
        tn=view(L.tn, B, torch.int32).clone(),
        state=view(L.state, B, torch.int32).clone(),
        nz=view(L.nz, B, torch.int32).clone(),
        fgsum=view(L.fgsum, B, torch.int64).clone(),
        xy=view(L.xy, B * cap * 2, torch.float32).view(B, cap, 2).clone(),
        dirs=view(L.dirs, B * K * cap * 2, torch.float32).view(B, K, cap, 2).clone(),
        hyp=view(L.hyp, B * K * hn * 2, torch.float32).view(B, K, hn, 2).clone(),
        counts=view(L.counts, B * K * hn, torch.int32).view(B, K, hn).clone(),
        win=view(L.win, B * K * 2, torch.float32).view(B, K, 2).clone(),
        capacity=cap,
    )
    return out


def _torch_rng_draws(mask, hn, K, min_num, max_num, select_mode, rounds=1):
    B, H, W = mask.shape
    dev = mask.device
    if select_mode == _lib.PVB_SELECT_BYTE:
        cur = mask.byte() if mask.dtype != torch.bool else mask.to(torch.uint8)
        fg = cur.sum(dim=(1, 2))
    else:
        cur = (mask == 1)
        fg = cur.sum(dim=(1, 2))
    fg_host = fg.tolist()
    selection = None
    idxs = torch.zeros((B, hn * rounds, K, 2), dtype=torch.int32, device=dev)
    for bi in range(B):
        if fg_host[bi] < min_num:
            continue
        sel_mask = cur[bi] != 0
        if fg_host[bi] > max_num:
            if selection is None:
                selection = torch.ones((B, H, W), dtype=torch.float32, device=dev)
            s = torch.zeros((H, W), dtype=torch.float32, device=dev).uniform_(0, 1)
            selection[bi] = s
            sel_mask = sel_mask & (s < (max_num / fg[bi].float()))
        tn = int(sel_mask.sum().item())
        if tn == 0:
            continue
        for r in range(rounds):
            idxs[bi, r * hn:(r + 1) * hn] = torch.zeros((hn, K, 2), dtype=torch.int32, device=dev).random_(0, tn)
    return idxs, selection


def _prep_optional(t, shape, dtype, name, device):
    if t is None:
        return None
    if not isinstance(t, torch.Tensor) or not t.is_cuda or t.device != device:
        raise RuntimeError(f"{name} must be a CUDA tensor on the same device")
    if tuple(t.shape) != tuple(shape):
        raise RuntimeError(f"{name} must have shape {tuple(shape)}, got {tuple(t.shape)}")
    return t.to(dtype).contiguous()


def _run(op, mask, vertex, hn, inlier_thresh, min_num, max_num, mean=None, idxs=None, selection=None,
         rng="philox", seed=None, img_base=0, capacity=None, debug=False, rounds=1, round_hn=None, exchange=None):
    mask, vertex = _check_inputs(mask, vertex)
    lib = _lib.load()
    dev = vertex.device
    B, H, W, K, _ = vertex.shape
    select_mode = _lib.PVB_SELECT_BYTE if op == "v3" else _lib.PVB_SELECT_EQ1
    if rng not in ("philox", "torch"):
        raise ValueError("rng must be 'philox' or 'torch'")
    with torch.cuda.device(dev):
        if rng == "torch" and idxs is None:
            idxs, sel = _torch_rng_draws(mask, round_hn or hn, K, min_num, max_num, select_mode, rounds)
            if selection is None:
                selection = sel
        idxs = _prep_optional(idxs, (B, hn, K, 2), torch.int32, "idxs", dev)
        selection = _prep_optional(selection, (B, H, W), torch.float32, "selection", dev)
        if seed is None:
            seed = _draw_seed() if (idxs is None or selection is None) else 0
        if capacity is None and selection is not None:
            capacity = H * W
        if capacity is not None and _VALIDATE_CAPACITY:
            need = H * W if selection is not None else min(H * W, int(max_num + 8 * math.sqrt(max(max_num, 0)) + 64))
            if int(capacity) < need:
                raise RuntimeError(f"capacity={capacity} cannot hold the selection (needs >= {need}; H*W is always safe)")
        d, nbytes = _cached_desc(lib, mask, vertex, hn, inlier_thresh, min_num, max_num, select_mode, seed, img_base, capacity)
        ws = _workspace(dev, nbytes)
        stream = torch.cuda.current_stream(dev).cuda_stream
        ip = idxs.data_ptr() if idxs is not None else None
        sp = selection.data_ptr() if selection is not None else None
        if op == "v3":
            out = torch.empty((B, K, 2), dtype=torch.float32, device=dev)
            if exchange is not None:
                _lib.check(lib.pvb_ransac_voting_v3_push(d, mask.data_ptr(), vertex.data_ptr(), ip, sp, out.data_ptr(),
                                                         ws.data_ptr(), ws.numel(), exchange[0], exchange[1], stream))
            elif B:
                _lib.check(lib.pvb_ransac_voting_v3(d, mask.data_ptr(), vertex.data_ptr(), ip, sp, out.data_ptr(),
                                                    ws.data_ptr(), ws.numel(), stream))
        else:
            if not isinstance(mean, torch.Tensor) or not mean.is_cuda or tuple(mean.shape) != (B, K, 2):
                raise RuntimeError("mean must be a CUDA tensor [b,vn,2]")
            mean_c = mean.float().contiguous()
            out = torch.empty((B, K, 2, 2), dtype=torch.float32, device=dev)
            if exchange is not None:
                _lib.check(lib.pvb_estimate_voting_distribution_push(d, mask.data_ptr(), vertex.data_ptr(), mean_c.data_ptr(),
                                                                     ip, sp, out.data_ptr(), ws.data_ptr(), ws.numel(),
                                                                     exchange[0], exchange[1], stream))
            elif B:
                _lib.check(lib.pvb_estimate_voting_distribution(d, mask.data_ptr(), vertex.data_ptr(),
                                                                mean_c.data_ptr(), ip, sp, out.data_ptr(),
                                                                ws.data_ptr(), ws.numel(), stream))
        if debug:
            if B:
                _lib.check(lib.pvb_read_status(d, ws.data_ptr(), stream))
            info = _views(ws, d, lib) if B else {}
            info["seed"] = seed
            return out, info
    return out


def ransac_voting_layer_v3(mask, vertex, round_hyp_num, inlier_thresh=0.999, confidence=0.99, max_iter=20,
                           min_num=5, max_num=30000, *, idxs=None, selection=None, rng="philox", seed=None,
                           img_base=0, capacity=None, debug=False, _exchange=None):
    del confidence, max_iter
    return _run("v3", mask, vertex, int(round_hyp_num), inlier_thresh, min_num, max_num, idxs=idxs,
                selection=selection, rng=rng, seed=seed, img_base=img_base, capacity=capacity, debug=debug,
                exchange=_exchange)


def ransac_voting_layer(mask, vertex, round_hyp_num, inlier_thresh=0.999, confidence=0.99, max_iter=20,
                        min_num=5, max_num=30000, **kw):
    return ransac_voting_layer_v3(mask, vertex, round_hyp_num, inlier_thresh, confidence, max_iter,
                                  min_num, max_num, **kw)


def estimate_voting_distribution_with_mean(mask, vertex, mean, round_hyp_num=256, min_hyp_num=4096, topk=128,
                                           inlier_thresh=0.99, min_num=5, max_num=30000, output_hyp=False, *,
                                           idxs=None, selection=None, rng="philox", seed=None, img_base=0,
                                           capacity=None, debug=False, _exchange=None):
    del topk, output_hyp
    rounds = int(math.ceil(min_hyp_num / round_hyp_num))
    hn = int(round_hyp_num) * rounds
    res = _run("dist", mask, vertex, hn, inlier_thresh, min_num, max_num, mean=mean, idxs=idxs,
               selection=selection, rng=rng, seed=seed, img_base=img_base, capacity=capacity, debug=debug,
               rounds=rounds, round_hn=int(round_hyp_num), exchange=_exchange)
    if debug:
        return mean, res[0], res[1]
    return mean, res


_host_scratch = {}


def ransac_voting_layer_v3_host(mask, vertex, round_hyp_num, inlier_thresh=0.999, confidence=0.99, max_iter=20,
                                min_num=5, max_num=30000, *, device=None, chunk_images=4, seed=None, img_base=0,
                                out=None, mode="auto"):
    del confidence, max_iter
    if mask.is_cuda or vertex.is_cuda:
        raise RuntimeError("ransac_voting_layer_v3_host takes host tensors")
    if vertex.dtype != torch.float32 or not vertex.is_contiguous() or not mask.is_contiguous():
        raise RuntimeError("host path needs contiguous float32 vertex and contiguous mask")
    if mask.dtype not in _MASK_DTYPES:
        raise RuntimeError(f"unsupported mask dtype {mask.dtype}")
    lib = _lib.load()
    dev = torch.device("cuda", torch.cuda.current_device()) if device is None else torch.device(device)
    B, H, W, K, _ = vertex.shape
    if seed is None:
        seed = _draw_seed()
    d = _make_desc(mask, vertex, int(round_hyp_num), inlier_thresh, min_num, max_num, _lib.PVB_SELECT_BYTE, seed,
                   img_base, None)
    chunk = max(1, min(int(chunk_images), B)) if B else 1
    if out is None:
        out = torch.empty((B, K, 2), dtype=torch.float32).pin_memory()
    if B == 0:
        return out
    with torch.cuda.device(dev):
        nbytes = lib.pvb_host_scratch_bytes(d, chunk)
        key = dev.index
        sc = _host_scratch.get(key)
        if sc is None or sc.numel() < nbytes:
            sc = torch.empty(nbytes + 256, dtype=torch.uint8, device=dev)
            _host_scratch[key] = sc
        flags = {"auto": 0, "inplace": _lib.PVB_HOST_INPLACE_MASK, "staged": _lib.PVB_HOST_STAGE_VERTEX}[mode]
        _lib.check(lib.pvb_ransac_voting_v3_host(d, mask.data_ptr(), vertex.data_ptr(), out.data_ptr(), chunk, flags,
                                                 sc.data_ptr(), sc.numel(),
                                                 torch.cuda.current_stream(dev).cuda_stream))
    return out


def install_as_reference_module():
    import importlib
    import importlib.util
    this = sys.modules[__name__]
    parent = None
    for name in ("lib", "lib.csrc", "lib.csrc.ransac_voting"):
        mod = sys.modules.get(name)
        if mod is None:
            try:
                found = importlib.util.find_spec(name) is not None
            except (ImportError, ValueError, AttributeError):
                found = False
            if found:
                mod = importlib.import_module(name)
            else:
                mod = types.ModuleType(name)
                mod.__path__ = []
                mod.__pvb_stand_in__ = True
                sys.modules[name] = mod
        if parent is not None and not hasattr(parent, name.rsplit(".", 1)[1]):
            setattr(parent, name.rsplit(".", 1)[1], mod)
        parent = mod
    sys.modules["lib.csrc.ransac_voting.ransac_voting_gpu"] = this
    sys.modules["lib.csrc.ransac_voting.ransac_voting"] = _ext
    parent.ransac_voting_gpu = this
    parent.ransac_voting = _ext
    return this
```

### include/pvnet_vote_b200.h

```cpp
#ifndef PVNET_VOTE_B200_H_
#define PVNET_VOTE_B200_H_

#include <stddef.h>
#include <stdint.h>

#ifdef __cplusplus
extern "C" {
#endif

#define PVB_VERSION 200

#if defined(__GNUC__)
#define PVB_API __attribute__((visibility("default")))
#else
#define PVB_API
#endif

typedef void *pvb_stream_t;

typedef enum pvb_status {
    PVB_OK = 0,
    PVB_ERR_INVALID = 1,
    PVB_ERR_CUDA = 2,
    PVB_ERR_WORKSPACE = 3,
    PVB_ERR_CAPACITY = 4,
    PVB_ERR_TIMEOUT = 5
} pvb_status;

typedef enum pvb_mask_dtype {
    PVB_MASK_U8 = 0,
    PVB_MASK_I8 = 1,
    PVB_MASK_I16 = 2,
    PVB_MASK_I32 = 3,
    PVB_MASK_I64 = 4,
    PVB_MASK_F32 = 5,
    PVB_MASK_F64 = 6
} pvb_mask_dtype;

typedef enum pvb_select_mode {
    PVB_SELECT_BYTE = 0,
    PVB_SELECT_EQ1 = 1
} pvb_select_mode;

typedef struct pvb_desc {
    int32_t B, H, W, K;
    int32_t hn;
    float inlier_thresh;
    int32_t min_num, max_num;
    int32_t mask_dtype;
    int32_t select_mode;
    int64_t mask_stride[3];
    int64_t vertex_stride[5];
    int32_t capacity;
    int32_t img_base;
    uint64_t seed;
    int32_t rng_tag_idx;
    int32_t rng_tag_sel;
} pvb_desc;

typedef struct pvb_layout {
    size_t total;
    size_t status;
    size_t fgsum;
    size_t nz;
    size_t tn;
    size_t state;
    size_t bits;
    size_t ticket;
    size_t blocktot;
    size_t xy;
    size_t dirs;
    size_t hyp;
    size_t counts;
    size_t win;
    size_t refit_partial;
    size_t refit_ticket;
    int32_t nwords;
    int32_t nblocks;
    int32_t capacity;
    int32_t refit_splits;
} pvb_layout;

PVB_API int pvb_version(void);
PVB_API const char *pvb_last_error(void);

PVB_API size_t pvb_workspace_bytes(const pvb_desc *d);
PVB_API int pvb_workspace_layout(const pvb_desc *d, pvb_layout *out);

PVB_API int pvb_ransac_voting_v3(const pvb_desc *d, const void *mask, const float *vertex,
                         const int32_t *idxs, const float *selection, float *out_kpt,
                         void *workspace, size_t workspace_bytes, pvb_stream_t stream);

PVB_API int pvb_decode_v3(const pvb_desc *d, const float *seg, int32_t classes, int64_t class_stride, int64_t *mask_out,
                          const float *vertex, const int32_t *idxs, const float *selection, float *out_kpt,
                          void *workspace, size_t workspace_bytes, pvb_stream_t stream);

PVB_API int pvb_estimate_voting_distribution(const pvb_desc *d, const void *mask, const float *vertex,
                                     const float *mean, const int32_t *idxs, const float *selection,
                                     float *out_cov, void *workspace, size_t workspace_bytes,
                                     pvb_stream_t stream);

PVB_API int pvb_uncertainty_weights(const float *cov, float *weights, int32_t n, pvb_stream_t stream);

typedef struct pvb_pnp_options {
    int32_t max_num_iterations;
    int32_t reserved;
    double function_tolerance;
    double gradient_tolerance;
    double parameter_tolerance;
} pvb_pnp_options;
PVB_API int pvb_uncertainty_pnp(const double *pts2d, const double *pts3d, const double *wgt2d, const double *K,
                                const double *init_rt, double *result_rt, int32_t *info, int32_t n, int32_t pn,
                                int64_t pts3d_stride, int64_t k_stride, const pvb_pnp_options *options, pvb_stream_t stream);

PVB_API int pvb_uncertainty_pnp_from_votes(const float *kpt_2d, const float *cov, const float *weights, const double *pts3d,
                                           const double *K, const double *init_rt, double *result_rt, double *init_out,
                                           float *weights_out, int32_t *info, int32_t n, int32_t pn, int64_t pts3d_stride,
                                           int64_t k_stride, const pvb_pnp_options *options, pvb_stream_t stream);

PVB_API int pvb_uncertainty_pnp_init(const double *pts2d, const double *pts3d, const double *wgt2d, const double *K,
                                     double *init_rt, int32_t n, int32_t pn, int64_t pts3d_stride, int64_t k_stride,
                                     pvb_stream_t stream);

PVB_API int pvb_read_status(const pvb_desc *d, const void *workspace, pvb_stream_t stream);

#define PVB_HOST_STAGE_VERTEX 2u
#define PVB_HOST_INPLACE_MASK 4u
PVB_API size_t pvb_host_scratch_bytes(const pvb_desc *d, int32_t chunk_images);
PVB_API int pvb_ransac_voting_v3_host(const pvb_desc *d, const void *mask_host, const float *vertex_host,
                              float *out_kpt_host, int32_t chunk_images, uint32_t flags,
                              void *dev_scratch, size_t dev_scratch_bytes, pvb_stream_t stream);

typedef struct pvb_exchange pvb_exchange;
#define PVB_IPC_HANDLE_BYTES 64
PVB_API int pvb_exchange_create(int32_t rank, int32_t world, int32_t slots, size_t bytes_per_rank, pvb_exchange **out);
PVB_API size_t pvb_exchange_bytes_per_rank(const pvb_exchange *ex);
PVB_API void *pvb_exchange_base(const pvb_exchange *ex);
PVB_API int pvb_exchange_get_handle(const pvb_exchange *ex, void *handle );
PVB_API int pvb_exchange_connect(pvb_exchange *ex, const void *handles );
PVB_API int pvb_exchange_connect_ptrs(pvb_exchange *ex, void *const *bases );
PVB_API int pvb_ransac_voting_v3_push(const pvb_desc *d, const void *mask, const float *vertex, const int32_t *idxs,
                                      const float *selection, float *out_kpt, void *workspace, size_t workspace_bytes,
                                      pvb_exchange *exchange, uint64_t seq, pvb_stream_t stream);
PVB_API int pvb_estimate_voting_distribution_push(const pvb_desc *d, const void *mask, const float *vertex, const float *mean,
                                                  const int32_t *idxs, const float *selection, float *out_cov, void *workspace,
                                                  size_t workspace_bytes, pvb_exchange *exchange, uint64_t seq,
                                                  pvb_stream_t stream);
PVB_API int pvb_exchange_wait(pvb_exchange *ex, uint64_t seq, void *out, const int32_t *floats_per_rank, double timeout_s,
                              pvb_stream_t stream);
PVB_API int pvb_exchange_status(pvb_exchange *ex, pvb_stream_t stream);
PVB_API int pvb_exchange_destroy(pvb_exchange *ex);

enum { PVB_STAGE_SELECT = 0,
       PVB_STAGE_GENERATE = 1,
       PVB_STAGE_VOTE = 2,
       PVB_STAGE_FINISH = 3,
       PVB_STAGE_COUNT = 4 };
PVB_API int pvb_profile_enable(int32_t every);
PVB_API int pvb_set_tuning(int32_t gather_mode, int32_t vote_variant);
PVB_API int pvb_profile_reset(void);
PVB_API int pvb_profile_read(double *ms, int32_t n);

PVB_API int pvb_generate_hypothesis(const float *direct, const float *coords, const int32_t *idxs, float *hyp,
                            int32_t tn, int32_t vn, int32_t hn, pvb_stream_t stream);
PVB_API int pvb_voting_for_hypothesis(const float *direct, const float *coords, const float *hyp, uint8_t *inliers,
                              int32_t tn, int32_t vn, int32_t hn, float inlier_thresh, pvb_stream_t stream);
PVB_API int pvb_generate_hypothesis_vanishing_point(const float *direct, const float *coords, const int32_t *idxs,
                                            float *hyp, int32_t tn, int32_t vn, int32_t hn,
                                            pvb_stream_t stream);
PVB_API int pvb_voting_for_hypothesis_vanishing_point(const float *direct, const float *coords, const float *hyp,
                                              uint8_t *inliers, int32_t tn, int32_t vn, int32_t hn,
                                              float inlier_thresh, pvb_stream_t stream);

PVB_API int pvb_vote_count(const float *direct, const float *coords, const float *hyp, int32_t *counts,
                   int32_t tn, int32_t vn, int32_t hn, float inlier_thresh,
                   void *workspace, size_t workspace_bytes, pvb_stream_t stream);
PVB_API size_t pvb_vote_count_workspace_bytes(int32_t tn, int32_t vn, int32_t hn);

#ifdef __cplusplus
}
#endif
#endif
```

Baseline: 224,500.

## Prune RANSAC hypotheses after voting on most tiles via bound-based survivor list

Adds a vote_prune_kernel that first counts votes for all hypotheses over about three quarters of the point tiles. The last block of that phase then publishes only the hypotheses whose partial count plus the remaining point count can still reach the current maximum. The remaining tiles vote only for those survivors, read through an acquire/release flag, with a fallback to all hypotheses when the list is not yet published. The aim is to cut vote work when hn exceeds 128, at the cost of extra workspace, cross-block synchronisation and counts that are no longer complete for pruned hypotheses. A FULL_COUNTS flag and a debug path keep the old behaviour.

```diff
diff --git a/clean_pvnet_b200/_lib.py b/clean_pvnet_b200/_lib.py
--- a/clean_pvnet_b200/_lib.py
+++ b/clean_pvnet_b200/_lib.py
@@ -9,6 +9,7 @@
 PVB_IPC_HANDLE_BYTES = 64
 (PVB_MASK_U8, PVB_MASK_I8, PVB_MASK_I16, PVB_MASK_I32, PVB_MASK_I64, PVB_MASK_F32, PVB_MASK_F64) = range(7)
 PVB_SELECT_BYTE, PVB_SELECT_EQ1 = 0, 1
+PVB_V3_FULL_COUNTS = 1
 
 
 class PvbDesc(ctypes.Structure):
@@ -29,7 +30,7 @@
 class PvbLayout(ctypes.Structure):
     _fields_ = [(n, ctypes.c_size_t) for n in
                 ("total", "status", "fgsum", "nz", "tn", "state", "bits", "ticket", "blocktot", "xy", "dirs", "hyp",
-                 "counts", "win", "refit_partial", "refit_ticket")] + [
+                 "counts", "win", "refit_partial", "refit_ticket", "vote_fallbacks", "vote_done", "vote_pub", "vote_surv")] + [
                     ("nwords", ctypes.c_int32), ("nblocks", ctypes.c_int32), ("capacity", ctypes.c_int32),
                     ("refit_splits", ctypes.c_int32)]
 
@@ -48,6 +49,8 @@
     "pvb_workspace_bytes": (_sz, [_dp]),
     "pvb_workspace_layout": (ctypes.c_int, [_dp, _lp]),
     "pvb_ransac_voting_v3": (ctypes.c_int, [_dp, _vp, _vp, _vp, _vp, _vp, _vp, _sz, _vp]),
+    "pvb_ransac_voting_v3_ex": (ctypes.c_int, [_dp, _vp, _vp, _vp, _vp, _vp, _vp, _sz, _vp, ctypes.c_uint64, ctypes.c_uint32,
+                                               _vp]),
     "pvb_decode_v3": (ctypes.c_int, [_dp, _vp, _i32, ctypes.c_int64, _vp, _vp, _vp, _vp, _vp, _vp, _sz, _vp]),
     "pvb_estimate_voting_distribution": (ctypes.c_int, [_dp, _vp, _vp, _vp, _vp, _vp, _vp, _vp, _sz, _vp]),
     "pvb_uncertainty_weights": (ctypes.c_int, [_vp, _vp, _i32, _vp]),
diff --git a/clean_pvnet_b200/csrc/api.cu b/clean_pvnet_b200/csrc/api.cu
--- a/clean_pvnet_b200/csrc/api.cu
+++ b/clean_pvnet_b200/csrc/api.cu
@@ -104,6 +104,9 @@
     L->refit_ticket = take(B * K * sizeof(int));
     L->ticket = take(B * sizeof(int));
     L->blocktot = take(B * nblocks * sizeof(int));
+    L->vote_fallbacks = take(sizeof(int));
+    L->vote_done = take(B * K * sizeof(int));
+    L->vote_pub = take(B * K * sizeof(int));
     L->bits = take(B * nwords * sizeof(uint32_t));
     L->xy = take(B * cap * sizeof(float2));
     L->dirs = take(B * K * cap * sizeof(float2));
@@ -111,6 +114,7 @@
     L->counts = take(B * K * hn * sizeof(int));
     L->win = take(B * K * sizeof(float2));
     L->refit_partial = take(B * K * splits * 5 * sizeof(double));
+    L->vote_surv = take(B * K * hn * sizeof(int));
     L->total = off;
     L->nwords = nwords;
     L->nblocks = nblocks;
@@ -125,6 +129,7 @@
     VoteArgs v;
     float2 *win;
     RefitScratch refit;
+    VotePrune prune;
 };
 
 int make_plan(const pvb_desc *d, const void *mask, const float *vertex, const int32_t *idxs,
@@ -171,6 +176,10 @@
     P->refit.partial = reinterpret_cast<double *>(w + L.refit_partial);
     P->refit.ticket = reinterpret_cast<int *>(w + L.refit_ticket);
     P->refit.splits = L.refit_splits;
+    P->prune.fallbacks = reinterpret_cast<int *>(w + L.vote_fallbacks);
+    P->prune.done = reinterpret_cast<int *>(w + L.vote_done);
+    P->prune.pub = reinterpret_cast<int *>(w + L.vote_pub);
+    P->prune.surv = reinterpret_cast<int *>(w + L.vote_surv);
     return PVB_OK;
 }
 
@@ -183,7 +192,7 @@
     return PVB_OK;
 }
 
-int run_front(const Plan &P, cudaStream_t st, ProfCall *pc)
+int run_front(const Plan &P, bool prune, cudaStream_t st, ProfCall *pc)
 {
     prof_start(pc, PVB_STAGE_SELECT, st);
     int rc = run_select(P, st);
@@ -194,7 +203,7 @@
     if (e != cudaSuccess) return cuda_fail(e, "generate kernel");
     prof_end(pc, PVB_STAGE_GENERATE, st);
     prof_start(pc, PVB_STAGE_VOTE, st);
-    e = launch_vote(P.v, false, st);
+    e = launch_vote(P.v, false, prune ? &P.prune : nullptr, st);
     if (e != cudaSuccess) return cuda_fail(e, "vote kernel");
     prof_end(pc, PVB_STAGE_VOTE, st);
     return PVB_OK;
@@ -262,8 +271,9 @@
 
 static int run_v3(const pvb_desc *d, const void *mask, const float *vertex, const int32_t *idxs, const float *selection,
                   float *out_kpt, void *workspace, size_t workspace_bytes, const float *seg, int32_t classes,
-                  int64_t class_stride, int64_t *mask_out, pvb_exchange *ex, uint64_t seq, cudaStream_t st)
-{
+                  int64_t class_stride, int64_t *mask_out, pvb_exchange *ex, uint64_t seq, uint32_t flags, cudaStream_t st)
+{
+    if (flags & ~(uint32_t)PVB_V3_FULL_COUNTS) return fail(PVB_ERR_INVALID, "unknown flags 0x%x", flags);
     Plan P;
     int rc = make_plan(d, seg ? static_cast<const void *>(seg) : mask, vertex, idxs, selection, workspace, workspace_bytes, 1u, 2u, &P);
     if (rc) return rc;
@@ -281,7 +291,7 @@
         P.s.mask_out = reinterpret_cast<long long *>(mask_out);
     }
     ProfCall *pc = prof_begin(true);
-    rc = run_front(P, st, pc);
+    rc = run_front(P, !(flags & PVB_V3_FULL_COUNTS), st, pc);
     if (rc) return rc;
     prof_start(pc, PVB_STAGE_FINISH, st);
     cudaError_t e = launch_refit(P.v, P.win, P.refit, out_kpt, pp, st);
@@ -294,7 +304,7 @@
                          const float *selection, float *out_kpt, void *workspace, size_t workspace_bytes,
                          pvb_stream_t stream)
 {
-    return run_v3(d, mask, vertex, idxs, selection, out_kpt, workspace, workspace_bytes, nullptr, 0, 0, nullptr, nullptr, 0,
+    return run_v3(d, mask, vertex, idxs, selection, out_kpt, workspace, workspace_bytes, nullptr, 0, 0, nullptr, nullptr, 0, 0u,
                   static_cast<cudaStream_t>(stream));
 }
 
@@ -304,7 +314,15 @@
 {
     if (!exchange) return fail(PVB_ERR_INVALID, "exchange is NULL");
     return run_v3(d, mask, vertex, idxs, selection, out_kpt, workspace, workspace_bytes, nullptr, 0, 0, nullptr, exchange, seq,
-                  static_cast<cudaStream_t>(stream));
+                  0u, static_cast<cudaStream_t>(stream));
+}
+
+PVB_API int pvb_ransac_voting_v3_ex(const pvb_desc *d, const void *mask, const float *vertex, const int32_t *idxs,
+                                    const float *selection, float *out_kpt, void *workspace, size_t workspace_bytes,
+                                    pvb_exchange *exchange, uint64_t seq, uint32_t flags, pvb_stream_t stream)
+{
+    return run_v3(d, mask, vertex, idxs, selection, out_kpt, workspace, workspace_bytes, nullptr, 0, 0, nullptr, exchange, seq,
+                  flags, static_cast<cudaStream_t>(stream));
 }
 
 PVB_API int pvb_decode_v3(const pvb_desc *d, const float *seg, int32_t classes, int64_t class_stride, int64_t *mask_out,
@@ -314,7 +332,7 @@
     if (classes < 1 || classes > 4096) return fail(PVB_ERR_INVALID, "classes must be in [1,4096]");
     if (!seg) return fail(PVB_ERR_INVALID, "seg is NULL");
     return run_v3(d, nullptr, vertex, idxs, selection, out_kpt, workspace, workspace_bytes, seg, classes, class_stride, mask_out,
-                  nullptr, 0, static_cast<cudaStream_t>(stream));
+                  nullptr, 0, 0u, static_cast<cudaStream_t>(stream));
 }
 
 static int run_distribution(const pvb_desc *d, const void *mask, const float *vertex, const float *mean, const int32_t *idxs,
@@ -333,7 +351,7 @@
         return PVB_OK;
     }
     ProfCall *pc = prof_begin(true);
-    rc = run_front(P, st, pc);
+    rc = run_front(P, false, st, pc);
     if (rc) return rc;
     prof_start(pc, PVB_STAGE_FINISH, st);
     cudaError_t e = launch_covariance(P.v, mean, out_cov, pp, st);
@@ -608,7 +626,7 @@
         PeerPush none;
         memset(&none, 0, sizeof(none));
         e = launch_generate(P.v, hp->cmp);
-        if (e == cudaSuccess) e = launch_vote(P.v, false, hp->cmp);
+        if (e == cudaSuccess) e = launch_vote(P.v, false, &P.prune, hp->cmp);
         if (e == cudaSuccess) e = launch_refit(P.v, P.win, P.refit, reinterpret_cast<float *>(sb + S.out), none, hp->cmp);
         if (e != cudaSuccess) return cuda_fail(e, "compute kernels");
         e = cudaMemcpyAsync(reinterpret_cast<char *>(out_kpt_host) + (size_t)b0 * obytes, sb + S.out, (size_t)c * obytes, cudaMemcpyDeviceToHost, hp->cmp);
@@ -626,7 +644,7 @@
 
 PVB_API int pvb_set_tuning(int32_t gather_mode, int32_t vote_variant)
 {
-    if (vote_variant < 0 || vote_variant > 3) return fail(PVB_ERR_INVALID, "vote_variant must be 0..3");
+    if (vote_variant < 0 || vote_variant > 4) return fail(PVB_ERR_INVALID, "vote_variant must be 0..4");
     if (gather_mode < 0 || gather_mode > 2) return fail(PVB_ERR_INVALID, "gather_mode must be 0..2");
     set_gather_tuning(gather_mode);
     set_vote_tuning(vote_variant);
@@ -747,7 +765,7 @@
     v.B = 1; v.K = vn; v.hn = hn; v.cap = tn; v.W = 0; v.H = 0; v.thresh = inlier_thresh;
     v.tn = meta; v.state = meta + 1; v.xy = xy;
     v.dirs = dirs; v.idxs = nullptr; v.hyp = hyp_k; v.counts = counts_k;
-    e = launch_vote(v, true, st);
+    e = launch_vote(v, true, nullptr, st);
     if (e != cudaSuccess) return cuda_fail(e, "vote kernel");
     e = launch_compat_unpack_counts(counts_k, counts, vn, hn, st);
     return e == cudaSuccess ? PVB_OK : cuda_fail(e, "unpack");
diff --git a/clean_pvnet_b200/csrc/kernels.h b/clean_pvnet_b200/csrc/kernels.h
--- a/clean_pvnet_b200/csrc/kernels.h
+++ b/clean_pvnet_b200/csrc/kernels.h
@@ -43,7 +43,13 @@
     int *counts;
 };
 cudaError_t launch_generate(const VoteArgs &a, cudaStream_t st);
-cudaError_t launch_vote(const VoteArgs &a, bool zero_counts, cudaStream_t st);
+struct VotePrune {
+    int *fallbacks;
+    int *done;
+    int *pub;
+    int *surv;
+};
+cudaError_t launch_vote(const VoteArgs &a, bool zero_counts, const VotePrune *prune, cudaStream_t st);
 void set_vote_tuning(int variant);
 void set_gather_tuning(int mode);
 struct RefitScratch { double *partial; int *ticket; int splits; };
diff --git a/clean_pvnet_b200/csrc/vote.cu b/clean_pvnet_b200/csrc/vote.cu
--- a/clean_pvnet_b200/csrc/vote.cu
+++ b/clean_pvnet_b200/csrc/vote.cu
@@ -64,33 +64,15 @@
     return ap - fabsf(pp);
 }
 
-template <int HPT, int NT, int MINB, int VOTE_TILE, int WS>
-__global__ void __launch_bounds__(NT, MINB)
-vote_kernel(const VoteK p)
+
+template <int NT, int VOTE_TILE>
+__device__ __forceinline__ void stage_tile(const float2 *__restrict__ dk, const float2 *__restrict__ xy, int n, int npad,
+                                           float kappa, float4 *s_a, float2 *s_b, float (*s_box)[NT / 32],
+                                           float &ox, float &oy, float &cmax)
 {
     constexpr int PPT = VOTE_TILE / NT;
     constexpr int NW = NT / 32;
-    constexpr int TEAM = WS * 32;
-    constexpr int TEAMS = NT / TEAM;
-    __shared__ __align__(16) float4 s_a[VOTE_TILE];
-    __shared__ __align__(16) float2 s_b[VOTE_TILE];
-    __shared__ float s_box[4][NW];
-    const VoteArgs &a = p.a;
-    const int b = blockIdx.z;
-    const int k = blockIdx.y % a.K, slice = blockIdx.y / a.K;
-    const int tn = min(a.tn[b], a.cap);
-    const int t0 = blockIdx.x * VOTE_TILE;
-    if (t0 >= tn) return;
-    const int n = min(VOTE_TILE, tn - t0);
-    const int npad = (n + VOTE_BLOCK - 1) / VOTE_BLOCK * VOTE_BLOCK;
     const int tid = threadIdx.x, lane = tid & 31, warp = tid >> 5;
-    const float kappa = p.cone.kappa, thresh = p.cone.thresh;
-    const float2 *hyp = a.hyp + ((size_t)b * a.K + k) * a.hn;
-    const float2 *xy = a.xy + (size_t)b * a.cap + t0;
-    const float2 *dk = a.dirs + ((size_t)b * a.K + k) * a.cap + t0;
-    const int team = tid / TEAM;
-    const int hbase = slice * (TEAM * HPT) + (tid - team * TEAM);
-
     float2 v[PPT], c[PPT];
     float x0 = CUDART_INF_F, x1 = -CUDART_INF_F, y0 = CUDART_INF_F, y1 = -CUDART_INF_F;
 #pragma unroll
@@ -113,8 +95,8 @@
     for (int w = 0; w < NW; ++w) {
         x0 = fminf(x0, s_box[0][w]); x1 = fmaxf(x1, s_box[1][w]); y0 = fminf(y0, s_box[2][w]); y1 = fmaxf(y1, s_box[3][w]);
     }
-    const float ox = 0.5f * (x0 + x1), oy = 0.5f * (y0 + y1);
-    const float cmax = (0.5f * (x1 - x0) + 0.5f * (y1 - y0)) * 1.000001f + 1e-3f;
+    ox = 0.5f * (x0 + x1); oy = 0.5f * (y0 + y1);
+    cmax = (0.5f * (x1 - x0) + 0.5f * (y1 - y0)) * 1.000001f + 1e-3f;
 
 #pragma unroll
     for (int r = 0; r < PPT; ++r) {
@@ -139,18 +121,109 @@
             s_a[i] = ra; s_b[i] = rb;
         }
     }
+}
+
+__device__ __forceinline__ void hyp_local(float2 q, float ox, float oy, float cmax, float band, float &xc, float &yc, float &d)
+{
+    xc = q.x - ox; yc = q.y - oy;
+    const float S = fabsf(xc) + fabsf(yc) + cmax;
+    d = fmaxf(band * S, 1e-30f);
+    if (!(S <= 1e15f) || !(d < CUDART_INF_F)) { xc = 0.f; yc = 0.f; d = CUDART_INF_F; }
+}
+
+template <int HPT, typename HypAt>
+__device__ __forceinline__ void score_block(uint32_t sa0, uint32_t sb0, const float4 *s_a, const float2 *s_b, int i0, int n,
+                                            const float (&hxc)[HPT], const float (&hyc)[HPT], const float (&dl)[HPT],
+                                            int (&neg)[HPT], const float2 *__restrict__ dk, const float2 *__restrict__ xy,
+                                            float thresh, HypAt hyp_at)
+{
+    const int lane = threadIdx.x & 31;
+    const uint32_t sa = sa0 + (uint32_t)i0 * 16u, sb = sb0 + (uint32_t)i0 * 8u;
+    float mn[HPT];
+#pragma unroll
+    for (int j = 0; j < HPT; ++j) mn[j] = CUDART_INF_F;
+#pragma unroll
+    for (int u = 0; u < VOTE_BLOCK; u += 2) {
+        const float4 ra0 = lds128(sa + u * 16), ra1 = lds128(sa + u * 16 + 16);
+        const float4 rbb = lds128(sb + u * 8);
+#pragma unroll
+        for (int j = 0; j < HPT; ++j) {
+            const float m0 = cone_margin(ra0, make_float2(rbb.x, rbb.y), hxc[j], hyc[j]);
+            const float m1 = cone_margin(ra1, make_float2(rbb.z, rbb.w), hxc[j], hyc[j]);
+            neg[j] += (int)(__float_as_uint(m0) >> 31);
+            neg[j] += (int)(__float_as_uint(m1) >> 31);
+            mn[j] = fminf(mn[j], fminf(fabsf(m0), fabsf(m1)));
+        }
+    }
+    bool flag = false;
+#pragma unroll
+    for (int j = 0; j < HPT; ++j) flag |= mn[j] < dl[j];
+    if (__any_sync(0xffffffffu, flag)) {
+        const int nb = min(VOTE_BLOCK, n - i0);
+        float4 ra = make_float4(0.f, 0.f, -1e30f, 0.f);
+        float2 rb = make_float2(0.f, 0.f), vv = make_float2(0.f, 0.f), cc = make_float2(0.f, 0.f);
+        if (lane < nb) {
+            ra = s_a[i0 + lane]; rb = s_b[i0 + lane];
+            vv = __ldg(dk + i0 + lane); cc = __ldg(xy + i0 + lane);
+        }
+#pragma unroll
+        for (int j = 0; j < HPT; ++j) {
+            unsigned bm = __ballot_sync(0xffffffffu, mn[j] < dl[j]);
+            while (bm) {
+                const int L = __ffs(bm) - 1;
+                bm &= bm - 1;
+                const float hx_ = __shfl_sync(0xffffffffu, hxc[j], L), hy_ = __shfl_sync(0xffffffffu, hyc[j], L);
+                const float dl_ = __shfl_sync(0xffffffffu, dl[j], L);
+                const float2 q = hyp_at(L, j);
+                int delta = 0;
+                if (lane < nb) {
+                    const float m = cone_margin(ra, rb, hx_, hy_);
+                    if (fabsf(m) < dl_) {
+                        const bool in = vote_exact(vv.x, vv.y, cc.x, cc.y, q.x, q.y, thresh);
+                        delta = (in ? 0 : 1) - (int)(__float_as_uint(m) >> 31);
+                    }
+                }
+                delta = __reduce_add_sync(0xffffffffu, delta);
+                if (lane == L) neg[j] += delta;
+            }
+        }
+    }
+}
+
+template <int HPT, int NT, int MINB, int VOTE_TILE, int WS>
+__global__ void __launch_bounds__(NT, MINB)
+vote_kernel(const VoteK p)
+{
+    constexpr int NW = NT / 32;
+    constexpr int TEAM = WS * 32;
+    constexpr int TEAMS = NT / TEAM;
+    __shared__ __align__(16) float4 s_a[VOTE_TILE];
+    __shared__ __align__(16) float2 s_b[VOTE_TILE];
+    __shared__ float s_box[4][NW];
+    const VoteArgs &a = p.a;
+    const int b = blockIdx.z;
+    const int k = blockIdx.y % a.K, slice = blockIdx.y / a.K;
+    const int tn = min(a.tn[b], a.cap);
+    const int t0 = blockIdx.x * VOTE_TILE;
+    if (t0 >= tn) return;
+    const int n = min(VOTE_TILE, tn - t0);
+    const int npad = (n + VOTE_BLOCK - 1) / VOTE_BLOCK * VOTE_BLOCK;
+    const int tid = threadIdx.x, lane = tid & 31;
+    const float2 *hyp = a.hyp + ((size_t)b * a.K + k) * a.hn;
+    const float2 *xy = a.xy + (size_t)b * a.cap + t0;
+    const float2 *dk = a.dirs + ((size_t)b * a.K + k) * a.cap + t0;
+    const int team = tid / TEAM;
+    const int hbase = slice * (TEAM * HPT) + (tid - team * TEAM);
+
+    float ox, oy, cmax;
+    stage_tile<NT, VOTE_TILE>(dk, xy, n, npad, p.cone.kappa, s_a, s_b, s_box, ox, oy, cmax);
 
     float hxc[HPT], hyc[HPT], dl[HPT];
     int neg[HPT];
 #pragma unroll
     for (int j = 0; j < HPT; ++j) {
         const int h = hbase + j * TEAM;
-        const float2 q = (h < a.hn) ? hyp[h] : make_float2(0.f, 0.f);
-        float xc = q.x - ox, yc = q.y - oy;
-        const float S = fabsf(xc) + fabsf(yc) + cmax;
-        float d = fmaxf(p.cone.band * S, 1e-30f);
-        if (!(S <= 1e15f) || !(d < CUDART_INF_F)) { xc = 0.f; yc = 0.f; d = CUDART_INF_F; }
-        hxc[j] = xc; hyc[j] = yc; dl[j] = d;
+        hyp_local((h < a.hn) ? hyp[h] : make_float2(0.f, 0.f), ox, oy, cmax, p.cone.band, hxc[j], hyc[j], dl[j]);
         neg[j] = 0;
     }
     __syncthreads();
@@ -160,57 +233,10 @@
     int mine = 0;
     for (int i0 = team * VOTE_BLOCK; i0 < npad; i0 += TEAMS * VOTE_BLOCK) {
         mine += VOTE_BLOCK;
-        const uint32_t sa = sa0 + (uint32_t)i0 * 16u, sb = sb0 + (uint32_t)i0 * 8u;
-        float mn[HPT];
-#pragma unroll
-        for (int j = 0; j < HPT; ++j) mn[j] = CUDART_INF_F;
-#pragma unroll
-        for (int u = 0; u < VOTE_BLOCK; u += 2) {
-            const float4 ra0 = lds128(sa + u * 16), ra1 = lds128(sa + u * 16 + 16);
-            const float4 rbb = lds128(sb + u * 8);
-#pragma unroll
-            for (int j = 0; j < HPT; ++j) {
-                const float m0 = cone_margin(ra0, make_float2(rbb.x, rbb.y), hxc[j], hyc[j]);
-                const float m1 = cone_margin(ra1, make_float2(rbb.z, rbb.w), hxc[j], hyc[j]);
-                neg[j] += (int)(__float_as_uint(m0) >> 31);
-                neg[j] += (int)(__float_as_uint(m1) >> 31);
-                mn[j] = fminf(mn[j], fminf(fabsf(m0), fabsf(m1)));
-            }
-        }
-        bool flag = false;
-#pragma unroll
-        for (int j = 0; j < HPT; ++j) flag |= mn[j] < dl[j];
-        if (__any_sync(0xffffffffu, flag)) {
-            const int nb = min(VOTE_BLOCK, n - i0);
-            float4 ra = make_float4(0.f, 0.f, -1e30f, 0.f);
-            float2 rb = make_float2(0.f, 0.f), vv = make_float2(0.f, 0.f), cc = make_float2(0.f, 0.f);
-            if (lane < nb) {
-                ra = s_a[i0 + lane]; rb = s_b[i0 + lane];
-                vv = __ldg(dk + i0 + lane); cc = __ldg(xy + i0 + lane);
-            }
-#pragma unroll
-            for (int j = 0; j < HPT; ++j) {
-                unsigned bm = __ballot_sync(0xffffffffu, mn[j] < dl[j]);
-                while (bm) {
-                    const int L = __ffs(bm) - 1;
-                    bm &= bm - 1;
-                    const float hx_ = __shfl_sync(0xffffffffu, hxc[j], L), hy_ = __shfl_sync(0xffffffffu, hyc[j], L);
-                    const float dl_ = __shfl_sync(0xffffffffu, dl[j], L);
-                    const int h = hbase - lane + L + j * TEAM;
-                    const float2 q = (h < a.hn) ? __ldg(hyp + h) : make_float2(0.f, 0.f);
-                    int delta = 0;
-                    if (lane < nb) {
-                        const float m = cone_margin(ra, rb, hx_, hy_);
-                        if (fabsf(m) < dl_) {
-                            const bool in = vote_exact(vv.x, vv.y, cc.x, cc.y, q.x, q.y, thresh);
-                            delta = (in ? 0 : 1) - (int)(__float_as_uint(m) >> 31);
-                        }
-                    }
-                    delta = __reduce_add_sync(0xffffffffu, delta);
-                    if (lane == L) neg[j] += delta;
-                }
-            }
-        }
+        score_block<HPT>(sa0, sb0, s_a, s_b, i0, n, hxc, hyc, dl, neg, dk, xy, p.cone.thresh, [&](int L, int j) {
+            const int h = hbase - lane + L + j * TEAM;
+            return (h < a.hn) ? __ldg(hyp + h) : make_float2(0.f, 0.f);
+        });
     }
     int *counts = a.counts + ((size_t)b * a.K + k) * a.hn;
 #pragma unroll
@@ -219,6 +245,125 @@
         const int cnt = mine - neg[j];
         if (h < a.hn && cnt) atomicAdd(counts + h, cnt);
     }
+}
+
+constexpr int PR_TILE = 512, PR_NT = 128, PR_HPT = 4, PR_GROUP = 32 * PR_HPT;
+
+__device__ __forceinline__ int ld_acquire(const int *p)
+{
+    int v;
+    asm volatile("ld.acquire.gpu.global.b32 %0, [%1];" : "=r"(v) : "l"(p) : "memory");
+    return v;
+}
+__device__ __forceinline__ void st_release(int *p, int v)
+{
+    asm volatile("st.release.gpu.global.b32 [%0], %1;" ::"l"(p), "r"(v) : "memory");
+}
+
+__global__ void __launch_bounds__(PR_NT, 8)
+vote_prune_kernel(const VoteK p, const VotePrune pr)
+{
+    constexpr int NT = PR_NT, NW = NT / 32, HPT = PR_HPT, TILE = PR_TILE, G = PR_GROUP;
+    __shared__ __align__(16) float4 s_a[TILE];
+    __shared__ __align__(16) float2 s_b[TILE];
+    __shared__ float s_box[4][NW];
+    __shared__ int s_pub;
+    const VoteArgs &a = p.a;
+    const int tid = threadIdx.x, lane = tid & 31, warp = tid >> 5;
+    const long long item = blockIdx.x;
+    const int Tcap = (a.cap + TILE - 1) / TILE, TAc = Tcap - Tcap / 4, TBc = Tcap / 4;
+    const long long BK = (long long)a.B * a.K;
+    const bool phase_a = item < BK * TAc;
+    long long bk;
+    int s;
+    if (phase_a) { bk = item / TAc; s = (int)(item - bk * TAc); }
+    else if (TBc > 0) { const long long j = item - BK * TAc; bk = j / TBc; s = (int)(j - bk * TBc); }
+    else return;
+    if (bk >= BK) return;
+    const int b = (int)(bk / a.K);
+    const int tn = min(a.tn[b], a.cap);
+    const int T = (tn + TILE - 1) / TILE, TA = T - T / 4;
+    const int tile = phase_a ? s : TA + s;
+    if (phase_a ? (s >= TA) : (tile >= T)) return;
+    if (!phase_a && tid == 0) {
+        const int v = ld_acquire(pr.pub + bk);
+        s_pub = v;
+        if (v == 0) atomicAdd(pr.fallbacks, 1);
+    }
+    const int t0 = tile * TILE;
+    const int n = min(TILE, tn - t0);
+    const int npad = (n + VOTE_BLOCK - 1) / VOTE_BLOCK * VOTE_BLOCK;
+    const float2 *hyp = a.hyp + bk * a.hn;
+    const float2 *xy = a.xy + (size_t)b * a.cap + t0;
+    const float2 *dk = a.dirs + bk * a.cap + t0;
+
+    float ox, oy, cmax;
+    stage_tile<NT, TILE>(dk, xy, n, npad, p.cone.kappa, s_a, s_b, s_box, ox, oy, cmax);
+    const int pubv = phase_a ? 0 : s_pub;
+    const int nh = pubv ? pubv - 1 : a.hn;
+    const int *list = pubv ? pr.surv + bk * a.hn : nullptr;
+    __syncthreads();
+
+    const uint32_t sa0 = (uint32_t)__cvta_generic_to_shared(s_a);
+    const uint32_t sb0 = (uint32_t)__cvta_generic_to_shared(s_b);
+    int *counts = a.counts + bk * a.hn;
+    auto hyp_index = [&](int pos) { return list ? __ldcg(list + pos) : pos; };
+    const int nblk = npad / VOTE_BLOCK;
+    const int P = ((nh + G - 1) / G) * nblk;
+    const int p0 = (int)((long long)P * warp / NW), p1 = (int)((long long)P * (warp + 1) / NW);
+    int g = p0 / nblk, blk = p0 - g * nblk;
+    float hxc[HPT], hyc[HPT], dl[HPT];
+    int neg[HPT];
+    int mine = 0;
+    for (int pi = p0; pi < p1;) {
+#pragma unroll
+        for (int j = 0; j < HPT; ++j) {
+            const int pos = g * G + lane + 32 * j;
+            hyp_local(pos < nh ? __ldg(hyp + hyp_index(pos)) : make_float2(0.f, 0.f), ox, oy, cmax, p.cone.band,
+                      hxc[j], hyc[j], dl[j]);
+            neg[j] = 0;
+        }
+        mine = 0;
+        for (; pi < p1 && blk < nblk; ++pi, ++blk) {
+            mine += VOTE_BLOCK;
+            score_block<HPT>(sa0, sb0, s_a, s_b, blk * VOTE_BLOCK, n, hxc, hyc, dl, neg, dk, xy, p.cone.thresh,
+                             [&](int L, int j) {
+                                 const int pos = g * G + L + 32 * j;
+                                 return pos < nh ? __ldg(hyp + hyp_index(pos)) : make_float2(0.f, 0.f);
+                             });
+        }
+#pragma unroll
+        for (int j = 0; j < HPT; ++j) {
+            const int pos = g * G + lane + 32 * j;
+            const int cnt = mine - neg[j];
+            if (pos < nh && cnt) atomicAdd(counts + hyp_index(pos), cnt);
+        }
+        ++g; blk = 0;
+    }
+
+    if (!phase_a || T == TA) return;
+    __threadfence();
+    __syncwarp();
+    int last = 0;
+    if (lane == 0) last = (atomicAdd(pr.done + bk, 1) == NW * TA - 1);
+    if (!__shfl_sync(0xffffffffu, last, 0)) return;
+    __threadfence();
+    const int R = tn - TA * TILE;
+    int mx = 0;
+    for (int h = lane; h < a.hn; h += 32) mx = max(mx, __ldcg(counts + h));
+    mx = __reduce_max_sync(0xffffffffu, mx);
+    int *surv = pr.surv + bk * a.hn;
+    int base = 0;
+    for (int h0 = 0; h0 < a.hn; h0 += 32) {
+        const int h = h0 + lane;
+        const bool keep = h < a.hn && __ldcg(counts + h) + R >= mx;
+        const unsigned bal = __ballot_sync(0xffffffffu, keep);
+        if (keep) surv[base + __popc(bal & ((1u << lane) - 1u))] = h;
+        base += __popc(bal);
+    }
+    __threadfence();
+    __syncwarp();
+    if (lane == 0) st_release(pr.pub + bk, base + 1);
 }
 
 ConeParams make_cone(float thresh)
@@ -243,7 +388,7 @@
 
 void set_vote_tuning(int variant) { g_vote_variant.store(variant, std::memory_order_relaxed); }
 
-cudaError_t launch_vote(const VoteArgs &a, bool zero_counts, cudaStream_t st)
+cudaError_t launch_vote(const VoteArgs &a, bool zero_counts, const VotePrune *prune, cudaStream_t st)
 {
     if (zero_counts) {
         cudaError_t e = cudaMemsetAsync(a.counts, 0, sizeof(int) * (size_t)a.B * a.K * a.hn, st);
@@ -253,6 +398,11 @@
     p.a = a;
     p.cone = make_cone(a.thresh);
     const int variant = g_vote_variant.load(std::memory_order_relaxed);
+    const long long items = (long long)a.B * a.K * ((a.cap + PR_TILE - 1) / PR_TILE);
+    if (prune && a.hn > 128 && variant <= 1 && items <= 0x7fffffffll) {
+        if (items > 0) vote_prune_kernel<<<(unsigned)items, PR_NT, 0, st>>>(p, *prune);
+        return cudaGetLastError();
+    }
 #define PVB_VOTE(HPT, NT, MINB, TILE, WS)                                               \
     do {                                                                                \
         const int slices = (a.hn + (HPT) * (WS) * 32 - 1) / ((HPT) * (WS) * 32);        \
diff --git a/clean_pvnet_b200/ransac_voting_gpu.py b/clean_pvnet_b200/ransac_voting_gpu.py
--- a/clean_pvnet_b200/ransac_voting_gpu.py
+++ b/clean_pvnet_b200/ransac_voting_gpu.py
@@ -184,7 +184,12 @@
         sp = selection.data_ptr() if selection is not None else None
         if op == "v3":
             out = torch.empty((B, K, 2), dtype=torch.float32, device=dev)
-            if exchange is not None:
+            if debug and (exchange is not None or B):
+                ex, seq = exchange if exchange is not None else (None, 0)
+                _lib.check(lib.pvb_ransac_voting_v3_ex(d, mask.data_ptr(), vertex.data_ptr(), ip, sp, out.data_ptr(),
+                                                       ws.data_ptr(), ws.numel(), ex, seq, _lib.PVB_V3_FULL_COUNTS,
+                                                       stream))
+            elif exchange is not None:
                 _lib.check(lib.pvb_ransac_voting_v3_push(d, mask.data_ptr(), vertex.data_ptr(), ip, sp, out.data_ptr(),
                                                          ws.data_ptr(), ws.numel(), exchange[0], exchange[1], stream))
             elif B:
diff --git a/include/pvnet_vote_b200.h b/include/pvnet_vote_b200.h
--- a/include/pvnet_vote_b200.h
+++ b/include/pvnet_vote_b200.h
@@ -75,6 +75,10 @@
     size_t win;
     size_t refit_partial;
     size_t refit_ticket;
+    size_t vote_fallbacks;
+    size_t vote_done;
+    size_t vote_pub;
+    size_t vote_surv;
     int32_t nwords;
     int32_t nblocks;
     int32_t capacity;
@@ -142,6 +146,10 @@
 PVB_API int pvb_ransac_voting_v3_push(const pvb_desc *d, const void *mask, const float *vertex, const int32_t *idxs,
                                       const float *selection, float *out_kpt, void *workspace, size_t workspace_bytes,
                                       pvb_exchange *exchange, uint64_t seq, pvb_stream_t stream);
+#define PVB_V3_FULL_COUNTS 1u
+PVB_API int pvb_ransac_voting_v3_ex(const pvb_desc *d, const void *mask, const float *vertex, const int32_t *idxs,
+                                    const float *selection, float *out_kpt, void *workspace, size_t workspace_bytes,
+                                    pvb_exchange *exchange, uint64_t seq, uint32_t flags, pvb_stream_t stream);
 PVB_API int pvb_estimate_voting_distribution_push(const pvb_desc *d, const void *mask, const float *vertex, const float *mean,
                                                   const int32_t *idxs, const float *selection, float *out_cov, void *workspace,
                                                   size_t workspace_bytes, pvb_exchange *exchange, uint64_t seq,
```

After: 226,300 (median of 6 runs). About the same (+0.8%).
